# decadenza/SimpleStereo

Measured on AMD Instinct MI355X. Metric: disparity MPixels/s (H*W*nDisp per second), higher is better.
Workload: dtype f32

## Files before the change

### simplestereo_amd/csrc/asw_exact_kernels.hip.h

```cpp
#pragma once
#include "asw_shared.hip.h"
#include "lab_kernels.hip.h"
#include "glibc_math.hip.h"

namespace ssamd {

struct AswExactArgs {
    const PixRec *recL, *recR;
    const double *labL, *labR;
    const double *prox;
    u64 *keyL, *keyR;
    int16_t *disp;
    AswExactQueue q;
    AswExactQueue raw;
    double *ecost;
    u64 *costL, *costR;
    uint32_t *idxL, *idxR;
    uint32_t *wslotL, *wslotR;
    uint32_t *wpix;
    double *wtab;
    unsigned int wcap;
    int H, W, win, pad, minD, maxD, row0, rows;
    double gammaC;
};

__device__ __forceinline__ double exact_sqrt(double x)
{
#pragma clang fp contract(off)
    const double y0 = sqrt(x);
    if (!(y0 > 0.0) || !(y0 < 1.0e300)) return y0;
    const double e = fma(-y0, y0, x);
    return y0 + e / (2.0 * y0);
}

__global__ __launch_bounds__(256) void bgr2lab_f64_pair_kernel(const PixRec *__restrict__ recL, const PixRec *__restrict__ recR,
                                                               double *__restrict__ labL, double *__restrict__ labR, long long npix)
{
    SSAMD_LAB_TABLES_IN_LDS(T)
    long long q = (long long)blockIdx.x * blockDim.x + threadIdx.x;
    const long long stride = (long long)gridDim.x * blockDim.x;
    for (; q < 2 * npix; q += stride) {
        const bool right = q >= npix;
        const long long p = right ? q - npix : q;
        const uint32_t v = (right ? recR : recL)[p].bgrx;
        double L, a, b;
        bgr_to_lab_f64(v & 0xff, (v >> 8) & 0xff, (v >> 16) & 0xff, L, a, b, T);
        double *const o = (right ? labR : labL) + 3 * p;
        o[0] = L; o[1] = a; o[2] = b;
    }
}

__device__ __forceinline__ bool exact_overflowed(const AswExactArgs &A)
{
    return A.q.counter[0] > A.q.cap || (A.raw.entries && A.raw.counter[0] > A.raw.cap);
}

__global__ __launch_bounds__(256) void asw_exact_filter_kernel(const AswExactArgs A)
{
    const unsigned n = min(A.raw.counter[0], A.raw.cap);
    const unsigned nloop = (n + 255u) & ~255u;
    for (unsigned e0 = blockIdx.x * blockDim.x; e0 < nloop; e0 += gridDim.x * blockDim.x) {
        const unsigned e = e0 + threadIdx.x;
        unsigned s2 = 0;
        uint32_t pix = 0, rkey = 0xffffffffu;
        int d = 0;
        if (e < n) {
            const u64 ent = A.raw.entries[e];
            const uint32_t key = A.raw.ekeys[e];
            rkey = key;
            pix = (uint32_t)ent;
            d = (int)((ent >> 32) & 0xffff);
            const unsigned sides = (unsigned)(ent >> 48) & 3u;
            const uint32_t esc = 0xC0000000u - __float_as_uint(2.0f * A.q.sat_abs);
            if (sides & EXACT_SIDE_L) {
                const u64 g = A.keyL[pix];
                if ((int)(uint32_t)g != d && (uint32_t)(g >> 32) < esc && exact_near(key, (uint32_t)(g >> 32), A.q.tol, A.q.sat_abs, exact_zkey(A.win))) s2 |= EXACT_SIDE_L;
            }
            if ((sides & EXACT_SIDE_R) && A.keyR) {
                const u64 g = A.keyR[pix - (uint32_t)d];
                if ((uint32_t)g != pix % (uint32_t)A.W && (uint32_t)(g >> 32) < esc && exact_near(key, (uint32_t)(g >> 32), A.q.tol, A.q.sat_abs, exact_zkey(A.win))) s2 |= EXACT_SIDE_R;
            }
        }
        asw_exact_push_wave(A.q, s2 != 0, pix, d, s2, rkey);
    }
}

__global__ __launch_bounds__(256) void asw_exact_escalate_kernel(const AswExactArgs A)
{
    const AswExactQueue &Q = A.q;
    const uint32_t esc = 0xC0000000u - __float_as_uint(2.0f * Q.sat_abs);
    const long long n = (long long)A.rows * A.W;
    for (long long q = (long long)blockIdx.x * blockDim.x + threadIdx.x; q < n; q += (long long)gridDim.x * blockDim.x) {
        const int x = (int)(q % A.W);
        const u64 gl = A.keyL[q];
        if (gl != KEY_NONE && (uint32_t)(gl >> 32) >= esc) {
            const int dwin = (int)(uint32_t)gl, dhi = min(A.maxD, x);
            const int cnt = dhi - A.minD;
            if (cnt > 0) {
                unsigned slot = atomicAdd(Q.counter, (unsigned)cnt);
                for (int d = A.minD; d <= dhi; ++d)
                    if (d != dwin) {
                        if (slot < Q.cap) Q.entries[slot] = exact_entry((uint32_t)q, d, EXACT_SIDE_L);
                        ++slot;
                    }
                Q.flagL[q] = 1;
            }
        }
        if (A.keyR) {
            const u64 gr = A.keyR[q];
            if (gr != KEY_NONE && (uint32_t)(gr >> 32) >= esc) {
                const int xwin = (int)(uint32_t)gr;
                const int dhi = min(A.maxD, A.W - 1 - x), cnt = dhi - A.minD;
                if (cnt > 0) {
                    unsigned slot = atomicAdd(Q.counter, (unsigned)cnt);
                    for (int d = A.minD; d <= dhi; ++d)
                        if (x + d != xwin) {
                            if (slot < Q.cap) Q.entries[slot] = exact_entry((uint32_t)(q + d), d, EXACT_SIDE_R);
                            ++slot;
                        }
                    Q.flagR[q] = 1;
                }
            }
        }
    }
}

static constexpr int EXACT_ZSEG = 64, EXACT_ZWIN_MAX = 64;
__global__ __launch_bounds__(256) void asw_exact_zero_kernel(const AswExactArgs A)
{
    extern __shared__ __attribute__((aligned(16))) char zsmem[];
    const AswExactQueue &Q = A.q;
    const int W = A.W, H = A.H, win = A.win, p = A.pad;
    const int segs_per_row = (W + EXACT_ZSEG - 1) / EXACT_ZSEG;
    const int tid = threadIdx.x;
    const int TW = EXACT_ZSEG + 2 * p;
    uint32_t *const tA = reinterpret_cast<uint32_t *>(zsmem);
    uint32_t *const tB = tA + win * TW;
    __shared__ int s_idx[EXACT_ZSEG], s_state[EXACT_ZSEG];
    __shared__ int s_cur;
    for (long long seg = blockIdx.x; seg < (long long)A.rows * segs_per_row; seg += gridDim.x) {
        const int yr = (int)(seg / segs_per_row), x0 = (int)(seg - (long long)yr * segs_per_row) * EXACT_ZSEG, y = A.row0 + yr;
        if (!Q.zrow[yr]) continue;
        for (int side = 0; side < (A.keyR ? 2 : 1); ++side) {
            __syncthreads();
            if (tid < EXACT_ZSEG) {
                const int x = x0 + tid;
                bool z = false;
                int idx = 0;
                if (x < W) {
                    const long long q = (long long)yr * W + x;
                    if (side == 0) {
                        z = Q.zeroL[q] != 0;
                        if (z) {
                            if (A.keyL) { const u64 g = A.keyL[q]; z = g != KEY_NONE && (uint32_t)(g >> 32) == 0u; idx = (int)(uint32_t)g; }
                            else idx = (int)A.disp[q];
                        }
                    } else {
                        z = Q.zeroR[q] != 0;
                        if (z) { const u64 g = A.keyR[q]; z = g != KEY_NONE && (uint32_t)(g >> 32) == 0u; idx = (int)(uint32_t)g; }
                    }
                }
                s_idx[tid] = idx;
                s_state[tid] = z ? 1 : 0;
            }
            if (__syncthreads_or(tid < EXACT_ZSEG && s_state[tid] == 1) == 0) continue;
            if (win >= EXACT_ZWIN_MAX) {
                if (tid < EXACT_ZSEG && s_state[tid] == 1) s_state[tid] = 3;
            } else {
                const PixRec *const imgA = side ? A.recR : A.recL, *const imgB = side ? A.recL : A.recR;
                auto stage = [&](uint32_t *tile, const PixRec *img, int shift) {
                    for (int k0 = 0; k0 < win * TW; k0 += 8 * 256) {
                        uint32_t v[8];
#pragma unroll
                        for (int u = 0; u < 8; ++u) {
                            const int k = k0 + u * 256 + tid, i = k / TW, c = k - i * TW, ii = y - p + i, cc = x0 - p + c + shift;
                            v[u] = (k < win * TW && (unsigned)ii < (unsigned)H && (unsigned)cc < (unsigned)W) ? img[(size_t)ii * W + cc].bgrx : 0x80000000u;
                        }
#pragma unroll
                        for (int u = 0; u < 8; ++u) {
                            const int k = k0 + u * 256 + tid;
                            if (k < win * TW) tile[k] = v[u];
                        }
                    }
                };
                stage(tA, imgA, 0);
                for (;;) {
                    __syncthreads();
                    if (tid == 0) {
                        int cur = -1;
                        for (int k = 0; k < EXACT_ZSEG; ++k)
                            if (s_state[k] == 1) { cur = side ? s_idx[k] - (x0 + k) : s_idx[k]; break; }
                        s_cur = cur;
                    }
                    __syncthreads();
                    const int d = s_cur;
                    if (d < 0) break;
                    const int shift = side ? d : -d;
                    stage(tB, imgB, shift);
                    __syncthreads();
                    const int px = tid & (EXACT_ZSEG - 1), part = tid >> 6;
                    const bool mine = s_state[px] == 1 && (side ? s_idx[px] - (x0 + px) : s_idx[px]) == d;
                    bool nz = false;
                    if (mine) {
                        uint32_t acc = 0;
                        for (int i = part; i < win; i += 4) {
                            const uint32_t *const ra = tA + i * TW + px, *const rb = tB + i * TW + px;
#pragma unroll 8
                            for (int j = 0; j < win; ++j) {
                                const uint32_t a = ra[j], b = rb[j];
                                acc |= ((a | b) >> 31) ? 0u : (a ^ b);
                            }
                        }
                        nz = acc != 0u;
                    }
                    __syncthreads();
                    if (mine && part == 0) s_state[px] = 2;
                    __syncthreads();
                    if (mine && nz) s_state[px] = 3;
                }
            }
            __syncthreads();
            if (tid < EXACT_ZSEG && s_state[tid] == 3) {
                const int xq = x0 + tid, widx = s_idx[tid];
                const long long pq = (long long)yr * W + xq;
                if (side == 0) {
                    const int dhi = min(A.maxD, xq), cnt = dhi - A.minD;
                    if (cnt > 0) {
                        unsigned slot = atomicAdd(Q.counter, (unsigned)cnt);
                        for (int d = A.minD; d <= dhi; ++d)
                            if (d != widx) { if (slot < Q.cap) Q.entries[slot] = exact_entry((uint32_t)pq, d, EXACT_SIDE_L); ++slot; }
                        Q.flagL[pq] = 1;
                    }
                } else {
                    const int dhi = min(A.maxD, W - 1 - xq), cnt = dhi - A.minD;
                    if (cnt > 0) {
                        unsigned slot = atomicAdd(Q.counter, (unsigned)cnt);
                        for (int d = A.minD; d <= dhi; ++d)
                            if (xq + d != widx) { if (slot < Q.cap) Q.entries[slot] = exact_entry((uint32_t)(pq + d), d, EXACT_SIDE_R); ++slot; }
                        Q.flagR[pq] = 1;
                    }
                }
            }
        }
    }
}

__device__ __forceinline__ void exact_assign_wslot(const AswExactArgs &A, bool flagged, u64 mask, uint32_t pix, uint32_t side)
{
    if (mask == 0 || A.wcap == 0) return;
    const int leader = (int)__builtin_ctzll(mask);
    const unsigned lane = __builtin_amdgcn_mbcnt_hi(~0u, __builtin_amdgcn_mbcnt_lo(~0u, 0u));
    unsigned base = 0;
    if ((int)lane == leader) base = atomicAdd(A.q.counter + 6, (unsigned)__builtin_popcountll(mask));
    base = (unsigned)__builtin_amdgcn_readlane((int)base, leader);
    if (flagged) {
        const unsigned slot = base + (unsigned)__builtin_popcountll(mask & (((u64)1 << lane) - 1));
        (side ? A.wslotR : A.wslotL)[pix] = slot;
        if (slot < A.wcap) A.wpix[slot] = pix | (side << 31);
    }
}

__global__ __launch_bounds__(256) void asw_exact_winners_kernel(const AswExactArgs A)
{
    const AswExactQueue &Q = A.q;
    const long long n = (long long)A.rows * A.W;
    for (long long q0 = (long long)blockIdx.x * blockDim.x; q0 < n; q0 += (long long)gridDim.x * blockDim.x) {
        const long long q = q0 + threadIdx.x;
        const bool inb = q < n;
        const bool fl = inb && Q.flagL[q];
        if (fl) {
            A.costL[q] = ~0ull;
            A.idxL[q] = 0xffffffffu;
        }
        const int dwin = fl ? (A.keyL ? (int)(uint32_t)A.keyL[q] : (int)A.disp[q]) : 0;
        const u64 ml = __builtin_amdgcn_ballot_w64(fl);
        if (ml && fl && (int)__builtin_ctzll(ml) == (int)(threadIdx.x & 63)) atomicAdd(Q.counter + 1, (unsigned)__builtin_popcountll(ml));
        exact_assign_wslot(A, fl, ml, (uint32_t)q, 0u);
        asw_exact_push_wave(Q, fl, (uint32_t)q, dwin, EXACT_SIDE_L, fl && A.keyL ? (uint32_t)(A.keyL[q] >> 32) : 0xffffffffu);
        if (A.keyR) {
            const bool fr = inb && Q.flagR[q];
            int xl = 0, xr = 0;
            if (fr) {
                A.costR[q] = ~0ull;
                A.idxR[q] = 0xffffffffu;
                xr = (int)(q % A.W);
                xl = (int)(uint32_t)A.keyR[q];
            }
            const u64 mr = __builtin_amdgcn_ballot_w64(fr);
            if (mr && fr && (int)__builtin_ctzll(mr) == (int)(threadIdx.x & 63)) atomicAdd(Q.counter + 2, (unsigned)__builtin_popcountll(mr));
            exact_assign_wslot(A, fr, mr, (uint32_t)q, 1u);
            asw_exact_push_wave(Q, fr, (uint32_t)(q + (xl - xr)), xl - xr, EXACT_SIDE_R, fr ? (uint32_t)(A.keyR[q] >> 32) : 0xffffffffu);
        }
    }
}

__global__ __launch_bounds__(256) void asw_exact_wtab_kernel(const AswExactArgs A)
{
#pragma clang fp contract(off)
    __shared__ uint64_t s_exp[256];
    for (int k = threadIdx.x; k < 256; k += blockDim.x) s_exp[k] = gm_exp_tab[k];
    __syncthreads();
    if (exact_overflowed(A)) return;
    const unsigned n = min(A.q.counter[6], A.wcap);
    const int lane = threadIdx.x & 63, W = A.W, H = A.H, win = A.win, p = A.pad, win2 = win * win;
    for (unsigned slot = blockIdx.x * 4 + (threadIdx.x >> 6); slot < n; slot += gridDim.x * 4) {
        const uint32_t pw = A.wpix[slot], pix = pw & 0x7fffffffu;
        const double *const lab = (pw >> 31) ? A.labR : A.labL;
        const int yr = (int)(pix / (uint32_t)W), x = (int)(pix - (uint32_t)yr * (uint32_t)W), y = A.row0 + yr;
        const double *const c = lab + 3 * ((size_t)y * W + x);
        const double c0 = c[0], c1 = c[1], c2 = c[2];
        double *const out = A.wtab + (size_t)slot * win2;
        for (int t = lane; t < win2; t += 64) {
            const int i = t / win, j = t - i * win, ii = y - p + i, cc = x - p + j;
            double w = 0.0;
            if ((unsigned)ii < (unsigned)H && (unsigned)cc < (unsigned)W) {
                const double *const tp = lab + 3 * ((size_t)ii * W + cc);
                const double a0 = tp[0] - c0, a1 = tp[1] - c1, a2 = tp[2] - c2;
                w = A.prox[t] * glibc_exp_t(-exact_sqrt(a0 * a0 + a1 * a1 + a2 * a2) / A.gammaC, s_exp);
            }
            out[t] = w;
        }
    }
}

static constexpr int EXACT_WAVES = 4;
static constexpr int EXACT_CHUNK = 256;
__global__ __launch_bounds__(64 * EXACT_WAVES) void asw_exact_eval_kernel(const AswExactArgs A)
{
#pragma clang fp contract(off)
    __shared__ double s_w[EXACT_WAVES][EXACT_CHUNK], s_c[EXACT_WAVES][EXACT_CHUNK];
    __shared__ uint64_t s_exp[256];
    for (int k = threadIdx.x; k < 256; k += blockDim.x) s_exp[k] = gm_exp_tab[k];
    __syncthreads();
    if (exact_overflowed(A)) return;
    const int lane = threadIdx.x & 63, wv = threadIdx.x >> 6;
    double *const sw = s_w[wv], *const sc = s_c[wv];
    const unsigned n = min(A.q.counter[0], A.q.cap);
    const int W = A.W, H = A.H, win = A.win, p = A.pad;
    for (unsigned e = blockIdx.x * EXACT_WAVES + wv; e < n; e += gridDim.x * EXACT_WAVES) {
        const u64 ent = A.q.entries[e];
        const uint32_t pix = (uint32_t)ent;
        const int d = (int)((ent >> 32) & 0xffff);
        const unsigned sides = (unsigned)(ent >> 48) & 3u;
        const int yr = (int)(pix / (uint32_t)W), x = (int)(pix - (uint32_t)yr * (uint32_t)W);
        const int y = A.row0 + yr, xr = x - d;
        const double *const cl = A.labL + 3 * ((size_t)y * W + x), *const cr = A.labR + 3 * ((size_t)y * W + xr);
        const double cl0 = cl[0], cl1 = cl[1], cl2 = cl[2], cr0 = cr[0], cr1 = cr[1], cr2 = cr[2];
        const int jlo = max(0, p - xr), jhi = min(win, W + p - x), ncol = jhi - jlo;
        const int ilo = max(0, p - y), ihi = min(win, H + p - y);
        const int ntap = (ihi - ilo) * ncol;
        const uint32_t s1 = A.wcap && A.q.flagL && A.q.flagL[pix] ? A.wslotL[pix] : 0xffffffffu;
        const uint32_t s2 = A.wcap && A.q.flagR && A.q.flagR[pix - (uint32_t)d] ? A.wslotR[pix - (uint32_t)d] : 0xffffffffu;
        const double *const t1 = s1 < A.wcap ? A.wtab + (size_t)s1 * win * win : nullptr;
        const double *const t2 = s2 < A.wcap ? A.wtab + (size_t)s2 * win * win : nullptr;
        double acc = 0.0;
        bool all_zero = false;
        if ((unsigned)(ent >> 48) & EXACT_HINT_ZERO) {
            bool nz = false;
            for (int t = lane; t < ntap; t += 64) {
                const int q = t / ncol, i = ilo + q, j = jlo + (t - q * ncol);
                const int ii = y - p + i, jj = xr - p + j, kk = x - p + j;
                nz = nz || __builtin_amdgcn_sad_u8(A.recL[(size_t)ii * W + kk].bgrx, A.recR[(size_t)ii * W + jj].bgrx, 0u) != 0u;
            }
            all_zero = __builtin_amdgcn_ballot_w64(nz) == 0;
        }
        for (int t0 = 0; t0 < (all_zero ? 0 : ntap); t0 += EXACT_CHUNK) {
            const int nt = min(EXACT_CHUNK, ntap - t0);
            for (int t = lane; t < nt; t += 64) {
                const int q = (t0 + t) / ncol, i = ilo + q, j = jlo + (t0 + t - q * ncol);
                const int ii = y - p + i, jj = xr - p + j, kk = x - p + j;
                const double pr = A.prox[i * win + j];
                double w1, w2;
                if (t1) w1 = t1[i * win + j];
                else {
                    const double *const tl = A.labL + 3 * ((size_t)ii * W + kk);
                    const double a0 = tl[0] - cl0, a1 = tl[1] - cl1, a2 = tl[2] - cl2;
                    w1 = pr * glibc_exp_t(-exact_sqrt(a0 * a0 + a1 * a1 + a2 * a2) / A.gammaC, s_exp);
                }
                if (t2) w2 = t2[i * win + j];
                else {
                    const double *const tr = A.labR + 3 * ((size_t)ii * W + jj);
                    const double b0 = tr[0] - cr0, b1 = tr[1] - cr1, b2 = tr[2] - cr2;
                    w2 = pr * glibc_exp_t(-exact_sqrt(b0 * b0 + b1 * b1 + b2 * b2) / A.gammaC, s_exp);
                }
                const int tad = min(40, (int)__builtin_amdgcn_sad_u8(A.recL[(size_t)ii * W + kk].bgrx, A.recR[(size_t)ii * W + jj].bgrx, 0u));
                const double ww = w1 * w2;
                sw[t] = ww;
                sc[t] = ww * tad;
            }
            __builtin_amdgcn_wave_barrier();
            asm volatile("s_waitcnt lgkmcnt(0)" ::: "memory");
            if (lane < 2) {
                const double *const src = lane ? sw : sc;
                int t = 0;
                for (; t + 16 <= nt; t += 16) {
                    double v[16];
#pragma unroll
                    for (int u = 0; u < 16; ++u) v[u] = src[t + u];
#pragma unroll
                    for (int u = 0; u < 16; ++u) acc += v[u];
                }
                for (; t < nt; ++t) acc += src[t];
            }
            asm volatile("s_waitcnt lgkmcnt(0)" ::: "memory");
            __builtin_amdgcn_wave_barrier();
        }
        const double tot = __shfl(acc, 1);
        if (lane == 0) {
            const double c = all_zero ? 0.0 : acc / tot;
            A.ecost[e] = c;
            const u64 bits = (u64)__double_as_longlong(c);
            if (sides & EXACT_SIDE_L) atomicMin(A.costL + pix, bits);
            if (sides & EXACT_SIDE_R) atomicMin(A.costR + (pix - (uint32_t)d), bits);
        }
    }
}

__global__ __launch_bounds__(256) void asw_exact_resolve_kernel(const AswExactArgs A)
{
    if (exact_overflowed(A)) return;
    const unsigned n = A.q.counter[0];
    for (unsigned e = blockIdx.x * blockDim.x + threadIdx.x; e < n; e += gridDim.x * blockDim.x) {
        const u64 ent = A.q.entries[e];
        const uint32_t pix = (uint32_t)ent;
        const int d = (int)((ent >> 32) & 0xffff);
        const unsigned sides = (unsigned)(ent >> 48) & 3u;
        const u64 bits = (u64)__double_as_longlong(A.ecost[e]);
        if ((sides & EXACT_SIDE_L) && A.costL[pix] == bits) atomicMin(A.idxL + pix, (uint32_t)d);
        if ((sides & EXACT_SIDE_R) && A.costR[pix - (uint32_t)d] == bits) atomicMin(A.idxR + (pix - (uint32_t)d), pix % (uint32_t)A.W);
    }
}

__global__ __launch_bounds__(256) void asw_exact_patch_kernel(const AswExactArgs A)
{
    if (exact_overflowed(A)) return;
    const long long n = (long long)A.rows * A.W;
    for (long long q = (long long)blockIdx.x * blockDim.x + threadIdx.x; q < n; q += (long long)gridDim.x * blockDim.x) {
        if (A.q.flagL[q] && A.idxL[q] != 0xffffffffu) {
            if (A.keyL) A.keyL[q] = (A.keyL[q] & 0xffffffff00000000ull) | (u64)A.idxL[q];
            else A.disp[q] = (int16_t)A.idxL[q];
        }
        if (A.keyR && A.q.flagR[q] && A.idxR[q] != 0xffffffffu) A.keyR[q] = (A.keyR[q] & 0xffffffff00000000ull) | (u64)A.idxR[q];
    }
}

}
```

### simplestereo_amd/csrc/asw_prepass_kernels.hip.h

```cpp
#pragma once
#include "common.hip.h"
#include "lab_kernels.hip.h"

namespace ssamd {

static constexpr int TADV_COLS = 64;
template <bool BYTES>
__device__ __forceinline__ void asw_tad_tile(const void *__restrict__ srcL, const void *__restrict__ srcR, unsigned char *__restrict__ evol,
                                             int W, int pad, int minD, int Dc, int Se, int erow0, int erows, int evolW, int rd, long long npix_total,
                                             int bx, int by, int bz, char *smem)
{
    uint32_t *const sL = reinterpret_cast<uint32_t *>(smem);
    uint32_t *const sR = sL + TADV_COLS;
    const int r = erow0 + by, z = bz, uc0 = bx * TADV_COLS;
    const int P = Se >> 2, dlo = minD + z * Dc, dhi = dlo + Dc - 1;
    const int u0 = uc0 - pad, xr0 = u0 - dhi;
    auto pixel = [&](const void *src, int col) -> uint32_t {
        const size_t q = (size_t)r * W + col;
        if constexpr (BYTES) {
            typedef uint32_t __attribute__((aligned(1))) u32_unaligned;
            const uint8_t *const b = reinterpret_cast<const uint8_t *>(src) + 3 * q;
            return (long long)q + 1 < npix_total ? (*reinterpret_cast<const u32_unaligned *>(b) & 0xffffffu)
                                                 : ((uint32_t)b[0] | ((uint32_t)b[1] << 8) | ((uint32_t)b[2] << 16));
        } else {
            return reinterpret_cast<const PixRec *>(src)[q].bgrx;
        }
    };
    for (int k = threadIdx.x; k < 2 * TADV_COLS + Dc; k += blockDim.x) {
        const bool isL = k < TADV_COLS;
        const int col = isL ? u0 + k : xr0 + (k - TADV_COLS);
        const uint32_t v = (unsigned)col < (unsigned)W ? pixel(isL ? srcL : srcR, col) : 0x80000000u;
        (isL ? sL : sR)[isL ? k : k - TADV_COLS] = v;
    }
    __syncthreads();
    const int ncols = min(TADV_COLS, evolW - uc0);
    uint32_t *const out = reinterpret_cast<uint32_t *>(evol + (((size_t)z * erows + by) * (size_t)evolW + uc0) * Se);
    auto dword = [&](int c, int slot, uint32_t lp) {
        uint32_t v = 0;
        const int d0 = rd == 6 ? 6 * (slot >> 1) + 4 * (slot & 1) : 4 * slot, nv = rd == 6 && (slot & 1) ? 2 : 4;
        if (!(lp >> 31) && d0 < Dc) {
            const uint32_t *const rp = sR + c + (Dc - 1) - d0;
#pragma unroll
            for (int q = 0; q < 4; ++q) {
                const uint32_t rv = q < nv && d0 + q < Dc ? rp[-q] : 0x80000000u;
                if (!(rv >> 31)) v |= min(__builtin_amdgcn_sad_u8(lp, rv, 0u), 40u) << (8 * q);
            }
        }
        return v;
    };
    if ((P & 3) == 0) {
        const int P4 = P >> 2;
        uint4 *const out4 = reinterpret_cast<uint4 *>(out);
        for (int k = threadIdx.x; k < ncols * P4; k += blockDim.x) {
            const int c = k / P4, s4 = 4 * (k - c * P4);
            const uint32_t lp = sL[c];
            out4[k] = make_uint4(dword(c, s4, lp), dword(c, s4 + 1, lp), dword(c, s4 + 2, lp), dword(c, s4 + 3, lp));
        }
        return;
    }
    for (int k = threadIdx.x; k < ncols * P; k += blockDim.x) {
        const int c = k / P, slot = k - c * P;
        out[k] = dword(c, slot, sL[c]);
    }
}

__global__ __launch_bounds__(256) void asw_tad_volume_kernel(const PixRec *__restrict__ recL, const PixRec *__restrict__ recR,
                                                             unsigned char *__restrict__ evol, int W, int pad, int minD, int Dc,
                                                             int Se, int erow0, int erows, int evolW, int rd = 4)
{
    extern __shared__ __attribute__((aligned(16))) char smem[];
    asw_tad_tile<false>(recL, recR, evol, W, pad, minD, Dc, Se, erow0, erows, evolW, rd, 0, blockIdx.x, blockIdx.y, blockIdx.z, smem);
}

struct AswPrepassArgs {
    const uint8_t *bgrL, *bgrR;
    PixRec *recL, *recR;
    unsigned char *evol;
    long long npix_total;
    int W, pad, minD, Dc, Se, erow0, erows, evolW, rd;
    int lab_blocks, ex, ey;
};
__global__ __launch_bounds__(256) void asw_prepass_kernel(const AswPrepassArgs P)
{
    extern __shared__ __attribute__((aligned(16))) char smem[];
    if ((int)blockIdx.x < P.lab_blocks) {
        SSAMD_LAB_TABLES_IN_LDS(T)
        const long long np = (long long)P.erows * P.W, first = (long long)P.erow0 * P.W;
        const uint8_t *const bl = P.bgrL + 3 * first, *const br = P.bgrR + 3 * first;
        PixRec *const rl = P.recL + first, *const rr = P.recR + first;
        typedef uint32_t __attribute__((aligned(1))) u32_unaligned;
        for (long long q = (long long)blockIdx.x * blockDim.x + threadIdx.x; q < 2 * np; q += (long long)P.lab_blocks * blockDim.x) {
            const bool right = q >= np;
            const long long p = right ? q - np : q;
            const uint8_t *const bgr = right ? br : bl;
            uint32_t B, G, R;
            if (p + 1 < np) {
                const uint32_t v = *reinterpret_cast<const u32_unaligned *>(bgr + 3 * p);
                B = v & 0xff; G = (v >> 8) & 0xff; R = (v >> 16) & 0xff;
            } else {
                B = bgr[3 * p]; G = bgr[3 * p + 1]; R = bgr[3 * p + 2];
            }
            PixRec o;
            bgr_to_lab(B, G, R, o.L, o.a, o.b, T);
            o.bgrx = B | (G << 8) | (R << 16);
            (right ? rr : rl)[p] = o;
        }
        return;
    }
    const int b = (int)blockIdx.x - P.lab_blocks, bx = b % P.ex, by = (b / P.ex) % P.ey, bz = b / (P.ex * P.ey);
    asw_tad_tile<true>(P.bgrL, P.bgrR, P.evol, P.W, P.pad, P.minD, P.Dc, P.Se, P.erow0, P.erows, P.evolW, P.rd, P.npix_total, bx, by, bz, smem);
}

}
```

### simplestereo_amd/csrc/host_asw.h

```cpp
namespace {
template <class T> int get_prox_table(TableCache &tc, const char *what, int win, double gammaP, hipStream_t s, const T **out)
{
    return get_table(tc, win, gammaP, (size_t)win * win, what, s, out, [&](T *host) {
        const int p = win / 2;
        for (int i = 0; i < win; ++i)
            for (int j = 0; j < win; ++j) {
                const double di = i - p, dj = j - p;
                host[(size_t)i * win + j] = (T)glibc_exp(-std::sqrt(di * di + dj * dj) / gammaP);
            }
    });
}
int get_prox(Ctx &c, int win, double gammaP, hipStream_t s, const float **out) { return get_prox_table(c.proxTabs, "proximity table", win, gammaP, s, out); }
int get_prox64(Ctx &c, int win, double gammaP, hipStream_t s, const double **out) { return get_prox_table(c.proxTabs64, "fp64 proximity table", win, gammaP, s, out); }

int reset_keys(DevBuf &keys, size_t nout, hipStream_t s)
{
    if (int rc = keys.reserve(nout * 8)) return rc;
    HIP_TRY(hipMemsetAsync(keys.ptr, 0xFF, nout * 8, s));
    return SSAMD_OK;
}

int launch_finalize(Ctx &c, int slot, bool lrcheck, int b0, int nb, int W, int16_t *d_disp, hipStream_t s,
                    int16_t *d_raw_right = nullptr)
{
    if (nb <= 0) return SSAMD_OK;
    const size_t off = (size_t)b0 * W;
    const long long n = (long long)nb * W;
    const int blocks = (int)std::min<long long>((n + 255) / 256, 256 * 8);
    Timed t(c, s, slot);
    if (d_raw_right) {
        hipLaunchKernelGGL(wta_decode_kernel, dim3(blocks), dim3(256), 0, s, (const u64 *)c.keyL.ptr + off, d_disp + off, nb, W, 0);
        hipLaunchKernelGGL(wta_decode_kernel, dim3(blocks), dim3(256), 0, s, (const u64 *)c.keyR.ptr + off, d_raw_right + off, nb, W, 1);
    } else if (lrcheck) {
        const size_t lds = (((size_t)W * 2 + 15) & ~(size_t)15) + W;
        int rc = grant_dyn_lds(c, (const void *)lr_check_fill_kernel, (int)lds);
        if (rc) return rc;
        hipLaunchKernelGGL(lr_check_fill_kernel, dim3(nb), dim3(256), lds, s, (const u64 *)c.keyL.ptr + off,
                           (const u64 *)c.keyR.ptr + off, d_disp + off, nb, W);
    } else {
        hipLaunchKernelGGL(wta_decode_kernel, dim3(blocks), dim3(256), 0, s, (const u64 *)c.keyL.ptr + off, d_disp + off, nb, W, 0);
    }
    HIP_TRY(hipGetLastError());
    return SSAMD_OK;
}

using AswKernel = void (*)(const AswArgs);
using AswWaveKernel = void (*)(const AswWaveArgs);
struct AswPipeVariant { bool costs; int SL, SR, Se; AswKernel kernel; };
const AswPipeVariant kPipeVariants[] = {
#define SSAMD_PIPE_INSTANCE(C, SL, SR, SE) {C, SL, SR, SE, asw_aggregate_pipe_kernel<C, SL, SR, SE>},
#include "asw_instances.inc"
#undef SSAMD_PIPE_INSTANCE
};
struct AswWaveVariant { int RD; bool costs; int RX, KL, KR, KM; bool creg; AswWaveKernel kernel; };
#define SSAMD_WAVE_VARIANT(RX, KL, KR, KM, CREG) {4, false, RX, KL, KR, KM, CREG, asw_aggregate_wave_kernel<false, RX, KL, KR, KM, CREG>}
const AswWaveVariant kWaveVariants[] = {
#define SSAMD_WAVE6_INSTANCE(C, K, CREG) {6, C, 4, 0, 0, K, CREG, asw_aggregate_wave6_kernel<C, K, CREG>},
#include "asw_instances.inc"
#undef SSAMD_WAVE6_INSTANCE
    SSAMD_WAVE_VARIANT(4, 0, 0, 2, false), SSAMD_WAVE_VARIANT(4, 0, 0, 2, true),
    SSAMD_WAVE_VARIANT(4, 0, 0, 3, false), SSAMD_WAVE_VARIANT(4, 0, 0, 3, true),
    SSAMD_WAVE_VARIANT(4, 0, 0, 4, false), SSAMD_WAVE_VARIANT(4, 0, 0, 4, true),
    SSAMD_WAVE_VARIANT(8, 0, 0, 2, false), SSAMD_WAVE_VARIANT(8, 0, 0, 3, false), SSAMD_WAVE_VARIANT(8, 0, 0, 4, false),
    SSAMD_WAVE_VARIANT(8, 2, 2, 0, false),
    SSAMD_WAVE_VARIANT(8, 1, 2, 0, false),
    SSAMD_WAVE_VARIANT(4, 1, 2, 0, false),
    SSAMD_WAVE_VARIANT(4, 2, 2, 0, false),
    SSAMD_WAVE_VARIANT(4, 2, 3, 0, false),
};
#undef SSAMD_WAVE_VARIANT

AswKernel asw_pick_pipe_kernel(const AswGeom &g, bool costs, int asw_static)
{
    AswKernel pk = nullptr;
    for (const AswPipeVariant &v : kPipeVariants) {
        if (v.costs != costs) continue;
        if (v.SL == 0 && !pk) pk = v.kernel;
        if (asw_static != 0 && v.SL == g.SL && v.SR == g.SR && v.Se == g.Se) pk = v.kernel;
    }
    return pk;
}

AswWaveKernel asw_pick_wave_kernel(const AswWaveGeom &g, bool costs, bool unrolled)
{
    const bool straight = unrolled && !costs;
    const int kl = g.merged ? 0 : (g.Txw + 63) / 64, kr = g.merged ? 0 : (g.nRcw + 63) / 64, km = g.merged ? g.K : 0;
    for (const AswWaveVariant &v : kWaveVariants)
        if (straight && v.RD == g.RD && !v.costs && v.RX == g.RX && v.KL == kl && v.KR == kr && v.KM == km && v.creg == (g.creg != 0)) return v.kernel;
    if (g.RD == 6) return costs ? asw_aggregate_wave6_kernel<true, 0> : asw_aggregate_wave6_kernel<false, 0>;
    return g.RX == 8 ? (costs ? asw_aggregate_wave_kernel<true, 8> : asw_aggregate_wave_kernel<false, 8>)
                     : (costs ? asw_aggregate_wave_kernel<true, 4> : asw_aggregate_wave_kernel<false, 4>);
}

struct MatchCall {
    const uint8_t *dL = nullptr, *dR = nullptr;
    const RemapSrc *rm = nullptr;
    int H = 0, W = 0, row0 = 0, rows = 0;
    int win = 0, maxD = 0, minD = 0;
    int16_t *d_disp = nullptr;
    hipStream_t s = nullptr;
};
struct AswCall : MatchCall {
    int skip_at = 0, skip = 0;
    double gammaC = 0, gammaP = 0;
    bool consistent = false, alternate = false, exact = false;
    float *d_costs = nullptr;
    int16_t *d_raw_right = nullptr;
};

AswCall asw_call(const uint8_t *dL, const uint8_t *dR, int H, int W, int row0, int rows, int win, int maxD, int minD, double gammaC,
                 double gammaP, int consistent, int16_t *d_disp, void *stream, bool alternate = false, bool exact = false)
{
    AswCall q;
    q.dL = dL; q.dR = dR; q.H = H; q.W = W; q.row0 = row0; q.rows = rows;
    q.win = win; q.maxD = maxD; q.minD = minD; q.gammaC = gammaC; q.gammaP = gammaP; q.consistent = consistent != 0;
    q.d_disp = d_disp; q.s = (hipStream_t)stream; q.alternate = alternate; q.exact = exact;
    return q;
}

struct AswRun : AswCall {
    Ctx &c;
    const Tuning &t;
    PlanOptions po;
    int p, nD, grows, r0, r1, lab_blocks;
    size_t nout;
    long long np2;
    ShapeKey shape;
    AswGeom geom;
    std::vector<AswGeom> trial;
    bool need_keys = false, lab_pending = false;
    size_t evol_cap_max = 0, evol_limit = 0;
    const float *d_prox = nullptr;
    const unsigned char *evol = nullptr;
    int evolW = 0;
    AswWaveGeom wave;
    AswExactQueue xq_final{}, xq_raw{}, xq_kernel{};
};

bool asw_is_direct(const AswRun &r, const AswGeom &g) { return r.nD >= 1 && (g.nchunks == 1 || g.wave_rx) && !r.consistent; }

int asw_check_call(const AswCall &q)
{
    int rc = check_common(q.H, q.W, q.win, q.minD, q.maxD, q.row0, q.rows);
    if (rc) return rc;
    if (q.skip < 0 || q.skip_at < 0 || q.skip_at + q.skip > q.rows) return fail(SSAMD_EINVAL, "bad row gap [%d,%d) in a range of %d rows", q.skip_at, q.skip_at + q.skip, q.rows);
    if (q.skip > 0 && (q.alternate || q.d_costs || q.d_raw_right)) return fail(SSAMD_EINVAL, "two row ranges: plain, consistent and exact matching only");
    if (q.skip == q.rows) return 1;
    if (!(q.gammaC > 0) || !(q.gammaP > 0)) return fail(SSAMD_EINVAL, "gammaC and gammaP must be positive");
    if (q.exact && (q.alternate || q.d_costs)) return fail(SSAMD_EINVAL, "the exact (fp64 tie-break) mode has no alternate-rows form and no cost dump");
    if (q.alternate && q.d_costs) return fail(SSAMD_EINVAL, "the alternate-rows mode has no cost dump");
    return q.rows == 0 ? 1 : SSAMD_OK;
}

bool asw_volume_fits(AswRun &r, size_t bytes)
{
    if (bytes > r.evol_cap_max) return false;
    if (bytes <= r.c.evol.cap) return true;
    if (!r.evol_limit) {
        size_t free_b = 0, total_b = 0;
        r.evol_limit = r.evol_cap_max;
        if (hipMemGetInfo(&free_b, &total_b) == hipSuccess) r.evol_limit = std::min(r.evol_cap_max, r.c.evol.cap + free_b / 2);
        else (void)hipGetLastError();
    }
    return bytes <= r.evol_limit;
}

bool asw_wave_volume_fits(AswRun &r, const AswGeom &g)
{
    AswWaveGeom wg;
    if (!g.wave_rx || !asw_wave_layout(wg, r.po, r.win, r.nD, g.wave_rx)) return !g.wave_rx;
    const int xt = (r.W + wg.Txw - 1) / wg.Txw, erows = std::min(r.H, r.row0 + r.rows + r.win / 2) - std::max(0, r.row0 - r.win / 2);
    return asw_volume_fits(r, (size_t)erows * (size_t)round_up(xt * wg.Txw + 2 * (r.win / 2), 4) * (size_t)wg.Se + 4096);
}

int asw_plan_call(AswRun &r)
{
    if (r.nD >= 1)
        if (int rc = asw_choose_geometry(r.geom, r.po, r.W, r.grows, r.win, r.nD)) return rc;
    const double call_taps = (double)r.W * r.grows * r.nD * r.win * r.win;
    if (autotune_due(g_asw_geom, r.shape, call_taps) && r.nD >= 1 && !asw_geometry_forced(r.t)) {
        AswGeom tmp;
        if (asw_search(tmp, r.po, r.W, r.grows, r.win, r.nD, &r.trial) != SSAMD_OK || r.trial.size() < 2) r.trial.clear();
    }
    r.evol_cap_max = r.t.evol_max_mb ? std::min((size_t)24 << 30, (size_t)r.t.evol_max_mb << 20) : (size_t)24 << 30;
    if (r.nD >= 1 && r.geom.wave_rx && !asw_wave_volume_fits(r, r.geom)) ++r.c.evol_fallbacks;
    if (r.nD >= 1 && !asw_wave_volume_fits(r, r.geom)) r.geom.wave_rx = 0;
    r.trial.erase(std::remove_if(r.trial.begin(), r.trial.end(), [&](const AswGeom &g) { return !asw_wave_volume_fits(r, g); }), r.trial.end());
    if (r.trial.size() < 2) r.trial.clear();
    r.need_keys = !asw_is_direct(r, r.geom) || r.alternate;
    for (const AswGeom &g : r.trial) r.need_keys = r.need_keys || !asw_is_direct(r, g);
    return SSAMD_OK;
}

int asw_lab_records(AswRun &r)
{
    Ctx &c = r.c;
    Timed t(c, r.s, SSAMD_K_LAB);
    if (r.rm)
        hipLaunchKernelGGL(remap_lab_records_pair_kernel, dim3(r.lab_blocks), dim3(256), 0, r.s, *r.rm, (PixRec *)c.recL.ptr, (PixRec *)c.recR.ptr,
                           (long long)r.r0 * r.W, r.np2);
    else
        hipLaunchKernelGGL(bgr2lab_records_pair_kernel, dim3(r.lab_blocks), dim3(256), 0, r.s, r.dL + (size_t)r.r0 * r.W * 3, r.dR + (size_t)r.r0 * r.W * 3,
                           (PixRec *)c.recL.ptr + (size_t)r.r0 * r.W, (PixRec *)c.recR.ptr + (size_t)r.r0 * r.W, r.np2);
    HIP_TRY(hipGetLastError());
    return SSAMD_OK;
}

int asw_prepare_volume(AswRun &r, const AswGeom &g)
{
    Ctx &c = r.c;
    hipStream_t s = r.s;
    r.evol = nullptr;
    int chunks = g.nchunks, Tx = g.Tx, Dc = g.Dc, Se = g.Se;
    if (g.wave_rx) {
        if (!asw_wave_layout(r.wave, r.po, r.win, r.nD, g.wave_rx, !r.d_costs && r.t.wave_unroll != 0))
            return fail(SSAMD_ELIMIT, "wave kernel geometry does not fit LDS");
        chunks = 1; Tx = r.wave.Txw; Dc = r.wave.Dc; Se = r.wave.Se;
    } else if (!g.pipe || r.t.asw_evol == 0) {
        return SSAMD_OK;
    }
    const int xt = (r.W + Tx - 1) / Tx, erows = r.r1 - r.r0;
    const int evolW = round_up(xt * Tx + 2 * r.p + (g.wave_rx ? 0 : Tx / 2 + 8), 4);
    const size_t bytes = (size_t)chunks * (size_t)erows * (size_t)evolW * (size_t)Se;
    if (c.evol.cap > ((size_t)256 << 20) && (bytes + 4096) * 4 < c.evol.cap) {
        if (r.trial.empty() && ++c.evol_small_calls >= 8) {
            (void)hipStreamSynchronize(s);
            c.evol.release();
            c.evol_small_calls = 0;
        }
    } else {
        c.evol_small_calls = 0;
    }
    int erc = SSAMD_ENOMEM;
    if (r.t.evol_fail) {
        void *none = nullptr;
        size_t free_b = 0, total_b = (size_t)512 << 30;
        (void)hipMemGetInfo(&free_b, &total_b);
        if (hipMalloc(&none, 2 * total_b) == hipSuccess) (void)hipFree(none);
    } else if (asw_volume_fits(r, bytes + 4096)) {
        erc = c.evol.reserve(bytes + 4096);
    }
    if (erc) {
        (void)hipGetLastError();
        if (g.wave_rx) return fail(erc == SSAMD_ENOMEM ? SSAMD_ENOMEM : erc, "TAD volume of %zu bytes does not fit the device memory left", bytes);
        ++c.evol_fallbacks;
        g_err.clear();
        return SSAMD_OK;
    }
    r.evol = (const unsigned char *)c.evol.ptr;
    r.evolW = evolW;
    const int rd = g.wave_rx ? r.wave.RD : 4;
    Timed t(c, s, SSAMD_K_LAB);
    const dim3 egrid((unsigned)((evolW + TADV_COLS - 1) / TADV_COLS), (unsigned)erows, (unsigned)chunks);
    const size_t elds = (size_t)(2 * TADV_COLS + Dc) * 4;
    const long long tiles = (long long)egrid.x * egrid.y * egrid.z;
    if (r.lab_pending && tiles + r.lab_blocks < (1ll << 31)) {
        AswPrepassArgs pa;
        pa.bgrL = r.dL; pa.bgrR = r.dR; pa.recL = (PixRec *)c.recL.ptr; pa.recR = (PixRec *)c.recR.ptr;
        pa.evol = (unsigned char *)c.evol.ptr; pa.npix_total = (long long)r.H * r.W;
        pa.W = r.W; pa.pad = r.p; pa.minD = r.minD; pa.Dc = Dc; pa.Se = Se; pa.erow0 = r.r0; pa.erows = erows; pa.evolW = evolW;
        pa.rd = rd;
        pa.lab_blocks = r.lab_blocks; pa.ex = (int)egrid.x; pa.ey = (int)egrid.y;
        if (int grc = grant_dyn_lds(c, (const void *)asw_prepass_kernel, (int)elds)) return grc;
        hipLaunchKernelGGL(asw_prepass_kernel, dim3((unsigned)(tiles + r.lab_blocks)), dim3(256), elds, s, pa);
        HIP_TRY(hipGetLastError());
        r.lab_pending = false;
        return SSAMD_OK;
    }
    if (r.lab_pending) {
        r.lab_pending = false;
        if (int lrc = asw_lab_records(r)) return lrc;
    }
    if (int grc = grant_dyn_lds(c, (const void *)asw_tad_volume_kernel, (int)elds)) return grc;
    hipLaunchKernelGGL(asw_tad_volume_kernel, egrid, dim3(256), elds, s, (const PixRec *)c.recL.ptr, (const PixRec *)c.recR.ptr,
                       (unsigned char *)c.evol.ptr, r.W, r.p, r.minD, Dc, Se, r.r0, erows, evolW, rd);
    HIP_TRY(hipGetLastError());
    return SSAMD_OK;
}

template <class Args> void asw_fill_args(Args &x, const AswRun &r, const AswGeom &g)
{
    const bool direct = asw_is_direct(r, g);
    x.recL = (const PixRec *)r.c.recL.ptr; x.recR = (const PixRec *)r.c.recR.ptr;
    x.prox = r.d_prox;
    x.keyL = direct ? nullptr : (u64 *)r.c.keyL.ptr;
    x.keyR = r.consistent ? (u64 *)r.c.keyR.ptr : nullptr;
    x.disp = direct ? r.d_disp : nullptr;
    x.costs = r.d_costs;
    x.cost_keys = 0;
    x.xq = r.xq_kernel;
    x.evol = r.evol; x.erow0 = r.r0; x.erows = r.r1 - r.r0; x.evolW = r.evolW;
    x.H = r.H; x.W = r.W; x.win = r.win; x.pad = r.p; x.minD = r.minD; x.maxD = r.maxD; x.row0 = r.row0; x.rows = r.rows;
    x.kC = (float)(-1.4426950408889634 / r.gammaC);
    x.ystep = r.alternate ? 2 : 1;
    x.yb0 = 0;
    x.yskip_at = r.skip > 0 ? r.skip_at : 0x7fffffff; x.yskip = r.skip;
}

int asw_launch_pipe(AswRun &r, const AswArgs &a, const dim3 &grid)
{
    Ctx &c = r.c;
    const AswGeom &g = a.g;
    const AswKernel pk = asw_pick_pipe_kernel(g, r.d_costs != nullptr, r.t.asw_static);
    const int pipe_lds = a.evol ? g.lds_bytes_evol : g.lds_bytes;
    if (pipe_lds > 160 * 1024) return fail(SSAMD_ELIMIT, "this tile needs the TAD volume (LDS %d bytes without it)", pipe_lds);
    if (int grc = grant_dyn_lds(c, (const void *)pk, pipe_lds)) return grc;
    int rows_main = r.grows;
    AswGeom tail_g;
    const int per_simd = (g.threads / 64 + 3) / 4;
    const long long resident = std::max(1, std::min(3 / std::max(1, per_simd), (160 * 1024) / std::max(1, pipe_lds)));
    const long long per_row = (long long)grid.x * g.nchunks, slots = (long long)c.cus * resident;
    if (!r.alternate && r.t.asw_tail != 0 && g.XG >= 4) {
        const long long n = per_row * r.grows;
        const long long full = n / slots, rem = n - full * slots;
        if (full >= 1 && rem > 0 && 2 * rem <= slots && (full < 32 || r.t.asw_tail > 0)) {
            const int rm = (int)(full * slots / per_row);
            if (rm >= 1 && rm < r.grows &&
                asw_layout_e(tail_g, r.po, r.win, (g.XG + 1) / 2, g.DG, 160 * 1024, g.JC, 8, true, false, true) && tail_g.pipe &&
                tail_g.Se == g.Se && tail_g.Dc == g.Dc &&
                (a.evol == nullptr || round_up(((r.W + tail_g.Tx - 1) / tail_g.Tx) * tail_g.Tx + 2 * r.p, 4) <= a.evolW)) {
                tail_g.nchunks = g.nchunks;
                rows_main = rm;
            }
        }
    }
    const long long items = per_row * rows_main;
    long long workers = r.t.asw_persist > 0 ? std::min<long long>(r.t.asw_persist, slots) : (r.t.asw_persist < 0 && items >= 64 * slots ? slots : 0);
    workers = std::min(workers, items);
    if (workers > 0 && items < (1ll << 30)) {
        const size_t pq_bytes = (size_t)(ASW_PQ_QUEUES + 1) * ASW_PQ_LINE * 4;
        if (!c.pq.ptr) {
            if (int prc = c.pq.reserve(pq_bytes)) return prc;
            HIP_TRY(hipMemsetAsync(c.pq.ptr, 0, pq_bytes, r.s));
        }
        HIP_TRY(hipMemsetAsync(c.pq.ptr, 0, (size_t)ASW_PQ_QUEUES * ASW_PQ_LINE * 4, r.s));
        AswArgs pa = a;
        pa.pq = (unsigned int *)c.pq.ptr;
        pa.pq_nx = (int)grid.x; pa.pq_ny = rows_main; pa.pq_items = (int)items;
        ++c.persist_launches;
        hipLaunchKernelGGL(pk, dim3((unsigned)workers), dim3(g.threads), pipe_lds, r.s, pa);
    } else {
        hipLaunchKernelGGL(pk, dim3(grid.x, rows_main, grid.z), dim3(g.threads), pipe_lds, r.s, a);
    }
    HIP_TRY(hipGetLastError());
    if (rows_main < r.grows) {
        ++c.tail_splits;
        AswArgs t = a;
        t.g = tail_g;
        t.yb0 = rows_main;
        const AswKernel tk = asw_pick_pipe_kernel(tail_g, r.d_costs != nullptr, 0);
        const int tail_lds = a.evol ? tail_g.lds_bytes_evol : tail_g.lds_bytes;
        if (int grc = grant_dyn_lds(c, (const void *)tk, tail_lds)) return grc;
        hipLaunchKernelGGL(tk, dim3((r.W + tail_g.Tx - 1) / tail_g.Tx, r.grows - rows_main, tail_g.nchunks), dim3(tail_g.threads),
                           tail_lds, r.s, t);
        HIP_TRY(hipGetLastError());
    }
    return SSAMD_OK;
}

int asw_launch(AswRun &r, const AswGeom &g)
{
    r.geom = g;
    if (g.wave_rx) {
        AswWaveArgs wa;
        asw_fill_args(wa, r, g);
        wa.g = r.wave;
        const AswWaveKernel wk = asw_pick_wave_kernel(wa.g, r.d_costs != nullptr, r.t.wave_unroll != 0);
        const int lds = wa.g.wave_lds * wa.g.waves, xt = (r.W + wa.g.Txw - 1) / wa.g.Txw;
        if (int grc = grant_dyn_lds(r.c, (const void *)wk, lds)) return grc;
        hipLaunchKernelGGL(wk, dim3((xt + wa.g.waves - 1) / wa.g.waves, r.grows, 1), dim3(64 * wa.g.waves), lds, r.s, wa);
        HIP_TRY(hipGetLastError());
        return SSAMD_OK;
    }
    AswArgs a{};
    asw_fill_args(a, r, g);
    a.g = g;
    const dim3 grid((r.W + g.Tx - 1) / g.Tx, r.grows, g.nchunks);
    if (g.pipe) return asw_launch_pipe(r, a, grid);
    const bool chunked = g.JC < r.win;
    AswKernel kern = chunked ? (r.d_costs ? asw_aggregate_kernel<true, true> : asw_aggregate_kernel<false, true>)
                             : (r.d_costs ? asw_aggregate_kernel<true, false> : asw_aggregate_kernel<false, false>);
    if (g.Rx == 4)
        kern = chunked ? (r.d_costs ? asw_aggregate_kernel<true, true, 4> : asw_aggregate_kernel<false, true, 4>)
                       : (r.d_costs ? asw_aggregate_kernel<true, false, 4> : asw_aggregate_kernel<false, false, 4>);
    if (int grc = grant_dyn_lds(r.c, (const void *)kern, g.lds_bytes)) return grc;
    hipLaunchKernelGGL(kern, grid, dim3(g.threads), g.lds_bytes, r.s, a);
    HIP_TRY(hipGetLastError());
    return SSAMD_OK;
}

int asw_autotune(AswRun &r)
{
    hipStream_t s = r.s;
    hipEvent_t e0 = nullptr, e1 = nullptr;
    HIP_TRY(hipEventCreate(&e0));
    HIP_TRY(hipEventCreate(&e1));
    bool all_prepared = true;
    const bool want_evol = r.t.asw_evol != 0;
    for (const AswGeom &g : r.trial) {
        if (asw_prepare_volume(r, g) != SSAMD_OK) { all_prepared = false; continue; }
        if (g.pipe && !g.wave_rx && want_evol && !r.evol) all_prepared = false;
        if (asw_launch(r, g) != SSAMD_OK) all_prepared = false;
    }
    const int fastest = autotune_rounds(r.trial.size(), 4, false, e0, e1, s, &all_prepared, [&](size_t ci) {
        const AswGeom &g = r.trial[ci];
        const bool launched = asw_prepare_volume(r, g) == SSAMD_OK && asw_launch(r, g) == SSAMD_OK;
        if (g.pipe && !g.wave_rx && want_evol && !r.evol) all_prepared = false;
        return launched;
    });
    if (fastest >= 0) r.geom = r.trial[fastest];
    (void)hipEventDestroy(e0);
    (void)hipEventDestroy(e1);
    if (all_prepared) autotune_keep(g_asw_geom, r.shape, r.geom);
    else g_err.clear();
    return SSAMD_OK;
}

int asw_final_volume(AswRun &r, AswGeom &final_geom)
{
    int rc = asw_prepare_volume(r, final_geom);
    if (rc == SSAMD_ENOMEM && final_geom.wave_rx) {
        ++r.c.evol_fallbacks;
        g_err.clear();
        final_geom.wave_rx = 0;
        r.geom = final_geom;
        if (!asw_is_direct(r, final_geom) && !r.need_keys) {
            if ((rc = reset_keys(r.c.keyL, r.nout, r.s))) return rc;
            r.need_keys = true;
        }
        rc = asw_prepare_volume(r, final_geom);
    }
    if (rc) return rc;
    if (final_geom.pipe && !final_geom.wave_rx && !r.evol && final_geom.lds_bytes > 160 * 1024) {
        AswGeom g2;
        if ((rc = asw_search(g2, PlanOptions{r.t, true}, r.W, r.grows, r.win, r.nD))) return rc;
        g2.wave_rx = 0;
        if (!asw_is_direct(r, g2) && !r.need_keys && (rc = reset_keys(r.c.keyL, r.nout, r.s))) return rc;
        final_geom = g2;
        if ((rc = asw_prepare_volume(r, final_geom))) return rc;
    }
    return SSAMD_OK;
}

int asw_alternate_fill(AswRun &r)
{
    Ctx &c = r.c;
    hipStream_t s = r.s;
    int rc;
    AswAltArgs f;
    const size_t nodd = (size_t)(r.rows / 2) * r.W;
    if ((double)nodd * ((r.nD + 7) / 8 + 1) >= 4.0e9)
        return fail(SSAMD_ELIMIT, "alternate-rows mode: image x disparity range too large for the 32-bit job counter");
    f.cap = (unsigned int)std::min<size_t>(std::max<size_t>(nodd, 1 << 16), 1u << 28);
    if (r.t.alt_queue_cap)
        f.cap = (unsigned int)r.t.alt_queue_cap;
    if ((rc = c.altq.reserve((size_t)f.cap * 8 + 16))) return rc;
    f.ctr = (unsigned int *)c.altq.ptr; f.queue = (u64 *)((char *)c.altq.ptr + 16);
    HIP_TRY(hipMemsetAsync(f.ctr, 0, 16, s));
    f.recL = (const PixRec *)c.recL.ptr; f.recR = (const PixRec *)c.recR.ptr; f.prox = r.d_prox;
    f.disp = r.d_disp; f.key = (u64 *)c.keyL.ptr;
    f.H = r.H; f.W = r.W; f.win = r.win; f.pad = r.p; f.minD = r.minD; f.maxD = r.maxD; f.row0 = r.row0; f.rows = r.rows;
    f.kC = (float)(-1.4426950408889634 / r.gammaC);
    const dim3 pix_grid((r.W + 255) / 256, r.rows / 2);
    Timed t(c, s, SSAMD_K_ASW_ALT);
    hipLaunchKernelGGL(asw_alt_scan_kernel, pix_grid, dim3(256), 0, s, f);
    hipLaunchKernelGGL(asw_alt_jobs_kernel, dim3(256 * 8), dim3(256), 0, s, f);
    hipLaunchKernelGGL(asw_alt_decode_kernel, pix_grid, dim3(256), 0, s, f);
    HIP_TRY(hipGetLastError());
    return SSAMD_OK;
}

int asw_device_impl(Ctx &c, const AswCall &q)
{
    int rc = asw_check_call(q);
    if (rc) return rc > 0 ? SSAMD_OK : rc;
    hipStream_t s = q.s;
    ScratchOrder order(c, s);
    const Tuning &t = tune();
    AswRun r{q, c, t, PlanOptions{t, false}};
    r.exact = q.exact && q.maxD >= q.minD;
    r.p = q.win / 2; r.nD = q.maxD - q.minD + 1;
    r.nout = (size_t)q.rows * q.W;
    r.grows = q.alternate ? (q.rows + 1) / 2 : q.rows - q.skip;
    r.shape = {q.W, r.grows, q.win, r.nD};
    r.r0 = std::max(0, q.row0 - r.p); r.r1 = std::min(q.H, q.row0 + q.rows + r.p);
    r.np2 = (long long)(r.r1 - r.r0) * q.W;
    r.lab_blocks = (int)std::min<long long>((2 * r.np2 + 255) / 256, 256 * 8);
    if ((rc = asw_plan_call(r))) return rc;
    if (r.need_keys && (rc = reset_keys(c.keyL, r.nout, s))) return rc;
    if (q.consistent && (rc = reset_keys(c.keyR, r.nout, s))) return rc;
    if (r.nD >= 1) {
        if ((rc = c.recL.reserve((size_t)q.H * q.W * sizeof(PixRec)))) return rc;
        if ((rc = c.recR.reserve((size_t)q.H * q.W * sizeof(PixRec)))) return rc;
        if ((rc = get_prox(c, q.win, q.gammaP, s, &r.d_prox))) return rc;
        r.lab_pending = r.trial.empty() && !q.rm && t.prepass_fuse != 0;
        if (!r.lab_pending && (rc = asw_lab_records(r))) return rc;
        if (!r.trial.empty() && (rc = asw_autotune(r))) return rc;
        AswGeom final_geom = r.geom;
        if ((rc = asw_final_volume(r, final_geom))) return rc;
        if (r.lab_pending) {
            r.lab_pending = false;
            if ((rc = asw_lab_records(r))) return rc;
        }
        if (r.exact) {
            if (!r.trial.empty()) {
                if (r.need_keys && (rc = reset_keys(c.keyL, r.nout, s))) return rc;
                if (q.consistent && (rc = reset_keys(c.keyR, r.nout, s))) return rc;
            }
            if ((rc = asw_exact_prepare(c, q.W, q.rows, q.win, r.nD, q.gammaC, q.consistent, asw_is_direct(r, final_geom), s, r.xq_final, r.xq_raw, r.xq_kernel))) return rc;
        }
        Timed agg(c, s, SSAMD_K_ASW_AGG);
        if ((rc = asw_launch(r, final_geom))) return rc;
    }
    const bool direct = asw_is_direct(r, r.geom);
    if (r.exact && r.nD >= 1 &&
        (rc = asw_exact_pass(c, r.xq_final, r.xq_raw, q.H, q.W, q.row0, q.rows, q.win, q.maxD, q.minD, q.gammaC, q.gammaP, q.consistent, direct, q.d_disp, s)))
        return rc;
    if (!direct && q.skip > 0) {
        if ((rc = launch_finalize(c, SSAMD_K_ASW_FIN, q.consistent, 0, q.skip_at, q.W, q.d_disp, s)) ||
            (rc = launch_finalize(c, SSAMD_K_ASW_FIN, q.consistent, q.skip_at + q.skip, q.rows - q.skip_at - q.skip, q.W, q.d_disp, s)))
            return rc;
    } else if (!direct && (rc = launch_finalize(c, SSAMD_K_ASW_FIN, q.consistent, 0, q.rows, q.W, q.d_disp, s, q.d_raw_right))) return rc;
    return q.alternate && q.rows > 1 ? asw_alternate_fill(r) : SSAMD_OK;
}

int asw_alternate_rows(Ctx &c, AswCall q, int row_parity)
{
    int rc = check_common(q.H, q.W, q.win, q.minD, q.maxD, q.row0, q.rows);
    if (rc) return rc;
    if (q.rows == 0) return SSAMD_OK;
    const int row0 = q.row0, rows = q.rows;
    const bool top_odd = ((row0 + row_parity) & 1) != 0, bottom_odd = ((row0 + rows - 1 + row_parity) & 1) != 0;
    if (top_odd && row0 == 0)
        return fail(SSAMD_EINVAL, "alternate rows: the first output row is an odd row of the image, the sub-image must start at least one row above it");
    const int e0 = top_odd ? row0 - 1 : row0, e1 = bottom_odd ? std::min(q.H, row0 + rows + 1) : row0 + rows;
    q.alternate = true;
    if (e0 == row0 && e1 == row0 + rows) return asw_device_impl(c, q);
    ScratchOrder order(c, q.s);
    if ((rc = c.altdisp.reserve((size_t)(e1 - e0) * q.W * 2))) return rc;
    int16_t *const d_disp = q.d_disp;
    q.row0 = e0; q.rows = e1 - e0; q.d_disp = (int16_t *)c.altdisp.ptr;
    if ((rc = asw_device_impl(c, q))) return rc;
    HIP_TRY(hipMemcpyAsync(d_disp, (const int16_t *)c.altdisp.ptr + (size_t)(row0 - e0) * q.W, (size_t)rows * q.W * 2, hipMemcpyDeviceToDevice, q.s));
    return SSAMD_OK;
}
}
```

### simplestereo_amd/csrc/host_asw_exact.h

```cpp
namespace {
int get_prox64(Ctx &c, int win, double gammaP, hipStream_t s, const double **out);

int asw_exact_prepare(Ctx &c, int W, int rows, int win, int nD, double gammaC, bool consistent, bool direct, hipStream_t s,
                      AswExactQueue &q, AswExactQueue &raw, AswExactQueue &kernel_q)
{
    const size_t nout = (size_t)rows * W;
    if (nout >= ((size_t)1 << 32)) return fail(SSAMD_ELIMIT, "exact mode: more than 2^32 output pixels per call");
    const size_t all_cands = 2 * (nout * (size_t)nD + nout);
    size_t cap = std::min<size_t>(std::max<size_t>(4 * nout, std::min<size_t>(all_cands, (size_t)1 << 23)), (size_t)1 << 26);
    if (tune().exact_cap) cap = (size_t)tune().exact_cap;
    size_t rawcap = direct ? 0 : std::min<size_t>(std::max<size_t>(2 * nout, std::min<size_t>(all_cands, (size_t)1 << 23)), (size_t)1 << 26);
    if (!direct && tune().exact_cap) rawcap = std::max<size_t>(rawcap, cap);
    if (!direct && tune().exact_rawcap) rawcap = (size_t)tune().exact_rawcap;
    int rc;
    if ((rc = c.xqueue.reserve(cap * 8)) || (rc = c.xcost.reserve(cap * 8)) || (rc = c.xflags.reserve(64 + 4 * nout + (size_t)rows)) ||
        (rc = c.xslots.reserve(nout * 32)) || (rawcap && (rc = c.xraw.reserve(rawcap * 12))))
        return rc;
    c.xcap = (unsigned int)cap;
    c.xrawcap = (unsigned int)rawcap;
    HIP_TRY(hipMemsetAsync(c.xflags.ptr, 0, 64 + 4 * nout + (size_t)rows, s));
    q.entries = (u64 *)c.xqueue.ptr;
    q.ekeys = nullptr;
    q.counter = (unsigned int *)c.xflags.ptr;
    q.flagL = (unsigned char *)c.xflags.ptr + 64;
    q.flagR = consistent ? q.flagL + nout : nullptr;
    q.zeroL = q.flagL + 2 * nout;
    q.zeroR = consistent ? q.flagL + 3 * nout : nullptr;
    q.zrow = q.flagL + 4 * nout;
    q.W = (unsigned int)W;
    q.cap = (unsigned int)cap;
    q.tol = (uint32_t)std::min(1.0e6, (double)tune().exact_tol * std::max(1.0, 5.0 / gammaC) * std::max(1.0, win / 35.0));
    q.sat_abs = (float)(1.5 * 2.0 * 2.0 * ((double)win * win + 3.0) * 1.1102230246251565e-16 * 40.0);
    q.deep = 0xffffffffu;
    raw = AswExactQueue{};
    if (!direct) {
        raw = q;
        union { float f; uint32_t u; } sa; sa.f = q.sat_abs;
        raw.deep = 0xC0000000u - sa.u;
        raw.entries = (u64 *)c.xraw.ptr;
        raw.ekeys = (uint32_t *)((u64 *)c.xraw.ptr + rawcap);
        raw.counter = q.counter + 4;
        raw.flagL = raw.flagR = nullptr;
        raw.cap = (unsigned int)rawcap;
    }
    kernel_q = direct ? q : raw;
    return SSAMD_OK;
}

int asw_exact_pass(Ctx &c, const AswExactQueue &q, const AswExactQueue &raw, int H, int W, int row0, int rows, int win, int maxD, int minD, double gammaC, double gammaP,
                   bool consistent, bool direct, int16_t *d_disp, hipStream_t s)
{
    const int p = win / 2;
    const size_t nout = (size_t)rows * W, npix = (size_t)H * W;
    int rc;
    const double *d_prox = nullptr;
    if ((rc = get_prox64(c, win, gammaP, s, &d_prox))) return rc;
    if ((rc = c.xlabL.reserve(npix * 24)) || (rc = c.xlabR.reserve(npix * 24))) return rc;
    AswExactArgs x;
    x.recL = (const PixRec *)c.recL.ptr; x.recR = (const PixRec *)c.recR.ptr;
    x.labL = (const double *)c.xlabL.ptr; x.labR = (const double *)c.xlabR.ptr;
    x.prox = d_prox;
    x.keyL = direct ? nullptr : (u64 *)c.keyL.ptr; x.keyR = consistent ? (u64 *)c.keyR.ptr : nullptr;
    x.disp = d_disp;
    x.q = q;
    x.raw = raw;
    x.ecost = (double *)c.xcost.ptr;
    x.costL = (u64 *)c.xslots.ptr; x.costR = x.costL + nout;
    x.idxL = (uint32_t *)(x.costR + nout); x.idxR = x.idxL + nout;
    x.wslotL = x.idxR + nout; x.wslotR = x.wslotL + nout;
    {
        const size_t per = (size_t)win * win * 8;
        size_t wcap = std::min<size_t>(65536, ((size_t)64 << 20) / per);
        if (nout >= ((size_t)1 << 31)) wcap = 0;
        if (wcap && (rc = c.xwtab.reserve(wcap * 8 + wcap * per))) return rc;
        x.wcap = (unsigned int)wcap;
        x.wpix = (uint32_t *)c.xwtab.ptr;
        x.wtab = (double *)((char *)c.xwtab.ptr + wcap * 8);
    }
    x.H = H; x.W = W; x.win = win; x.pad = p; x.minD = minD; x.maxD = maxD; x.row0 = row0; x.rows = rows;
    x.gammaC = gammaC;
    Timed t(c, s, SSAMD_K_ASW_EXACT);
    {
        const int r0 = std::max(0, row0 - p), r1 = std::min(H, row0 + rows + p);
        const long long np2 = (long long)(r1 - r0) * W;
        const int blocks = (int)std::min<long long>((2 * np2 + 255) / 256, 256 * 8);
        hipLaunchKernelGGL(bgr2lab_f64_pair_kernel, dim3(blocks), dim3(256), 0, s, x.recL + (size_t)r0 * W, x.recR + (size_t)r0 * W,
                           (double *)c.xlabL.ptr + 3 * (size_t)r0 * W, (double *)c.xlabR.ptr + 3 * (size_t)r0 * W, np2);
    }
    const int pb = (int)std::min<long long>(((long long)nout + 255) / 256, 256 * 8);
    if (raw.entries) {
        hipLaunchKernelGGL(asw_exact_filter_kernel, dim3(256 * 8), dim3(256), 0, s, x);
        hipLaunchKernelGGL(asw_exact_escalate_kernel, dim3(pb), dim3(256), 0, s, x);
    }
    {
        const int zwin = std::min(win, EXACT_ZWIN_MAX - 1);
        const size_t zlds = (size_t)2 * zwin * (EXACT_ZSEG + 2 * (zwin / 2)) * 4;
        if ((rc = grant_dyn_lds(c, (const void *)asw_exact_zero_kernel, (int)zlds))) return rc;
        const long long segs = (long long)rows * ((W + EXACT_ZSEG - 1) / EXACT_ZSEG);
        hipLaunchKernelGGL(asw_exact_zero_kernel, dim3((unsigned)std::min<long long>(segs, 256 * 64)), dim3(256), zlds, s, x);
    }
    hipLaunchKernelGGL(asw_exact_winners_kernel, dim3(pb), dim3(256), 0, s, x);
    if (x.wcap) hipLaunchKernelGGL(asw_exact_wtab_kernel, dim3(256 * 4), dim3(256), 0, s, x);
    hipLaunchKernelGGL(asw_exact_eval_kernel, dim3((unsigned)(c.cus * 5)), dim3(64 * EXACT_WAVES), 0, s, x);
    hipLaunchKernelGGL(asw_exact_resolve_kernel, dim3(256 * 4), dim3(256), 0, s, x);
    hipLaunchKernelGGL(asw_exact_patch_kernel, dim3(pb), dim3(256), 0, s, x);
    HIP_TRY(hipGetLastError());
    ++c.exact_calls;
    return SSAMD_OK;
}

int asw_exact_counters(Ctx &c, unsigned int (&ctr)[5])
{
    std::fill(ctr, ctr + 5, 0u);
    if (!c.xflags.ptr || c.exact_calls == 0) return SSAMD_OK;
    HIP_TRY(hipDeviceSynchronize());
    HIP_TRY(hipMemcpy(ctr, c.xflags.ptr, sizeof(ctr), hipMemcpyDeviceToHost));
    return SSAMD_OK;
}
}
```

### simplestereo_amd/csrc/host_context.h

```cpp
namespace {
thread_local std::string g_err;

int fail(int code, const char *fmt, ...)
{
    char buf[512];
    va_list ap;
    va_start(ap, fmt);
    vsnprintf(buf, sizeof(buf), fmt, ap);
    va_end(ap);
    g_err = buf;
    return code;
}

#include "ssamd_options.h"
#include "asw_plan.h"
#include "gsw_plan.h"
#include "ftp_plan.h"
#include "np_unwrap_plan.h"

std::mutex g_tune_mutex;
std::atomic<unsigned> g_tune_version{1};

std::map<std::string, std::string> g_tuning_env;
Tuning tuning_from_env()
{
    Tuning t;
    for (const char *n : kTuningNames)
        if (const char *v = getenv(n)) {
            g_tuning_env[n] = v;
            (void)tuning_assign(t, n, v);
        }
    return t;
}
Tuning g_tuning = tuning_from_env();

const Tuning &tune()
{
    thread_local Tuning snap;
    thread_local unsigned seen = 0;
    const unsigned v = g_tune_version.load(std::memory_order_acquire);
    if (v != seen) {
        std::lock_guard<std::mutex> lk(g_tune_mutex);
        snap = g_tuning;
        seen = v;
    }
    return snap;
}

#define HIP_TRY(expr)                                                                              \
    do {                                                                                           \
        hipError_t e_ = (expr);                                                                    \
        if (e_ != hipSuccess)                                                                      \
            return fail(e_ == hipErrorOutOfMemory ? SSAMD_ENOMEM : SSAMD_EHIP, "%s failed: %s",    \
                        #expr, hipGetErrorString(e_));                                             \
    } while (0)

struct DevBuf {
    void *ptr = nullptr;
    size_t cap = 0;
    int reserve(size_t bytes)
    {
        if (bytes <= cap) return SSAMD_OK;
        if (ptr) { (void)hipFree(ptr); ptr = nullptr; cap = 0; }
        size_t want = bytes + bytes / 8 + 256;
        hipError_t e = hipMalloc(&ptr, want);
        if (e != hipSuccess) {
            ptr = nullptr;
            (void)hipGetLastError();
            return fail(SSAMD_ENOMEM, "hipMalloc(%zu) failed: %s", want, hipGetErrorString(e));
        }
        cap = want;
        return SSAMD_OK;
    }
    void release()
    {
        if (ptr) (void)hipFree(ptr);
        ptr = nullptr; cap = 0;
    }
};

struct Profile {
    bool on = false;
    struct Pair { hipEvent_t a, b; int slot; };
    std::vector<Pair> pending;
    std::vector<hipEvent_t> pool;
    double ms[SSAMD_K_COUNT] = {0};
    long long n[SSAMD_K_COUNT] = {0};
    hipEvent_t get()
    {
        if (!pool.empty()) { hipEvent_t e = pool.back(); pool.pop_back(); return e; }
        hipEvent_t e = nullptr;
        (void)hipEventCreate(&e);
        return e;
    }
    void drain()
    {
        for (auto &p : pending) {
            float t = 0.f;
            if (hipEventSynchronize(p.b) == hipSuccess && hipEventElapsedTime(&t, p.a, p.b) == hipSuccess) {
                ms[p.slot] += t;
                n[p.slot] += 1;
            }
            pool.push_back(p.a);
            pool.push_back(p.b);
        }
        pending.clear();
    }
};

struct TableEntry {
    int k0 = 0; double k1 = 0;
    DevBuf dev;
    std::vector<unsigned char> host;
};
struct TableCache {
    std::list<TableEntry> entries;
    size_t max_entries;
    explicit TableCache(size_t n) : max_entries(n) {}
    TableEntry *find(int k0, double k1)
    {
        for (auto it = entries.begin(); it != entries.end(); ++it)
            if (it->k0 == k0 && it->k1 == k1) {
                entries.splice(entries.begin(), entries, it);
                return &entries.front();
            }
        return nullptr;
    }
};

struct Ctx {
    std::mutex mu;
    int dev = -1;
    int cus = 256;
    bool lut_ready = false;
    hipStream_t stream = nullptr;
    DevBuf imgL, imgR, recL, recR, keyL, keyR, disp, costs, lab, altq, evol, altdisp;
    DevBuf xlabL, xlabR, xflags, xqueue, xcost, xslots, xctr, xraw, xwtab;
    DevBuf pq;
    DevBuf uwIn, uwOut;
    DevBuf ftpBand, ftpPhase;
    std::map<int, DevBuf> ftpTabs;
    DevBuf ftpRefTab;
    bool ftpRefTabReady = false;
    int32_t *ftpBandHost = nullptr;
    size_t ftpBandHostCap = 0;
    hipEvent_t ftp_band_copied = nullptr;
    unsigned int xcap = 0, xrawcap = 0;
    TableCache proxTabs{8}, gswTabs{4}, proxTabs64{8};
    std::map<const void *, int> max_dyn_lds;
    hipEvent_t scratch_free = nullptr;
    int evol_small_calls = 0;
    long long evol_fallbacks = 0;
    long long tail_splits = 0;
    long long exact_calls = 0;
    long long persist_launches = 0;
    long long gsw_plain_calls = 0;
    Profile prof;
};

Ctx g_ctx[16];

struct DeviceGuard {
    int saved = -1;
    DeviceGuard() { if (hipGetDevice(&saved) != hipSuccess) saved = -1; }
    ~DeviceGuard() { if (saved >= 0) (void)hipSetDevice(saved); }
    DeviceGuard(const DeviceGuard &) = delete;
    DeviceGuard &operator=(const DeviceGuard &) = delete;
};

struct Timed {
    Ctx &c; hipStream_t s; int slot; hipEvent_t a = nullptr, b = nullptr;
    Timed(Ctx &c_, hipStream_t s_, int slot_) : c(c_), s(s_), slot(slot_)
    {
        if (c.prof.on) { a = c.prof.get(); b = c.prof.get(); (void)hipEventRecord(a, s); }
    }
    ~Timed()
    {
        if (a) { (void)hipEventRecord(b, s); c.prof.pending.push_back({a, b, slot}); }
    }
};

struct CtxLock {
    DeviceGuard guard;
    std::unique_lock<std::mutex> lk;
    Ctx *c = nullptr;
    Ctx *operator->() { return c; }
    Ctx &operator*() { return *c; }
};

int get_ctx(int device, CtxLock &out)
{
    int n = 0;
    if (hipGetDeviceCount(&n) != hipSuccess || n <= 0)
        return fail(SSAMD_ENODEVICE, "no HIP device visible: libssamd has no CPU fallback");
    if (device < 0) device = out.guard.saved >= 0 ? out.guard.saved : 0;
    if (device >= n || device >= 16) return fail(SSAMD_EINVAL, "device ordinal %d out of range (%d visible)", device, n);
    HIP_TRY(hipSetDevice(device));
    Ctx &c = g_ctx[device];
    out.lk = std::unique_lock<std::mutex>(c.mu);
    out.c = &c;
    if (c.dev < 0) {
        c.dev = device;
        int cus = 0;
        if (hipDeviceGetAttribute(&cus, hipDeviceAttributeMultiprocessorCount, device) == hipSuccess && cus > 0) c.cus = cus;
        else (void)hipGetLastError();
        HIP_TRY(hipStreamCreateWithFlags(&c.stream, hipStreamNonBlocking));
        HIP_TRY(hipEventCreateWithFlags(&c.scratch_free, hipEventDisableTiming));
    }
    if (!c.lut_ready) {
        float lut[256];
        for (int v = 0; v < 256; ++v) {
            float x = v / 255.0;
            if (x > 0.04045) x = glibc_powf_pos((float)((x + 0.055) / 1.055), (float)2.4);
            else x /= 12.92;
            x *= 100;
            lut[v] = x;
        }
        HIP_TRY(hipMemcpyToSymbol(HIP_SYMBOL(c_lin100), lut, sizeof(lut)));
        c.lut_ready = true;
    }
    return SSAMD_OK;
}

int grant_dyn_lds(Ctx &c, const void *kernel, int bytes)
{
    int &granted = c.max_dyn_lds[kernel];
    if (bytes <= granted || bytes <= 48 * 1024) return SSAMD_OK;
    HIP_TRY(hipFuncSetAttribute(kernel, hipFuncAttributeMaxDynamicSharedMemorySize, bytes));
    granted = bytes;
    return SSAMD_OK;
}

struct ScratchOrder {
    Ctx &c; hipStream_t s;
    ScratchOrder(Ctx &c_, hipStream_t s_) : c(c_), s(s_) { (void)hipStreamWaitEvent(s, c.scratch_free, 0); }
    ~ScratchOrder() { (void)hipEventRecord(c.scratch_free, s); }
};

int check_common(int H, int W, int win, int minD, int maxD, int row0, int rows)
{
    if (H <= 0 || W <= 0) return fail(SSAMD_EINVAL, "Wrong image dimensions!");
    if (!(win > 0 && win % 2 == 1)) return fail(SSAMD_EINVAL, "winSize must be a positive odd number!");
    if (minD < 0) return fail(SSAMD_EINVAL, "minDisparity must be >= 0 (negative values are undefined behaviour in the reference)");
    if (W > 32767 || maxD > 32767) return fail(SSAMD_ELIMIT, "width / maxDisparity exceed the int16 disparity range");
    if (row0 < 0 || rows < 0 || row0 + rows > H) return fail(SSAMD_EINVAL, "output row range [%d,%d) outside the image (height %d)", row0, row0 + rows, H);
    if (win > 255) return fail(SSAMD_ELIMIT, "winSize %d > 255 not supported", win);
    if (rows > 65535) return fail(SSAMD_ELIMIT, "more than 65535 output rows per call: split the image into row strips");
    return SSAMD_OK;
}

template <class T, class Fill>
int get_table(TableCache &tc, int k0, double k1, size_t n, const char *what, hipStream_t s, const T **out, Fill fill)
{
    if (TableEntry *e = tc.find(k0, k1)) { *out = (const T *)e->dev.ptr; return SSAMD_OK; }
    if (tc.entries.size() >= tc.max_entries) {
        HIP_TRY(hipDeviceSynchronize());
        (void)hipFree(tc.entries.back().dev.ptr);
        tc.entries.pop_back();
    }
    tc.entries.emplace_front();
    TableEntry &e = tc.entries.front();
    e.k0 = k0; e.k1 = k1;
    e.host.resize(n * sizeof(T));
    fill(reinterpret_cast<T *>(e.host.data()));
    int rc = e.dev.reserve(n * sizeof(T));
    if (rc) { tc.entries.pop_front(); return rc; }
    hipError_t he = hipMemcpyAsync(e.dev.ptr, e.host.data(), n * sizeof(T), hipMemcpyHostToDevice, s);
    if (he != hipSuccess) {
        (void)hipFree(e.dev.ptr);
        tc.entries.pop_front();
        return fail(SSAMD_EHIP, "hipMemcpyAsync(%s) failed: %s", what, hipGetErrorString(he));
    }
    *out = (const T *)e.dev.ptr;
    return SSAMD_OK;
}

struct HostIn { DevBuf Ctx::*buf; const void *host; size_t bytes; size_t at = 0; };
struct HostOut { DevBuf Ctx::*buf; void *host; size_t bytes; size_t at = 0; };
inline char *staged(Ctx &c, DevBuf Ctx::*buf, size_t at = 0) { return (char *)(c.*buf).ptr + at; }

template <class Launch>
int host_route(int device, std::initializer_list<HostIn> in, const HostOut &out, Launch launch)
{
    CtxLock c;
    int rc = get_ctx(device, c);
    if (rc) return rc;
    for (const HostIn &i : in)
        if ((rc = ((*c).*i.buf).reserve(i.at + i.bytes))) return rc;
    if ((rc = ((*c).*out.buf).reserve(out.at + out.bytes))) return rc;
    hipStream_t s = c->stream;
    ScratchOrder order(*c, s);
    for (const HostIn &i : in) HIP_TRY(hipMemcpyAsync(staged(*c, i.buf, i.at), i.host, i.bytes, hipMemcpyHostToDevice, s));
    if ((rc = launch(*c, s))) return rc;
    HIP_TRY(hipMemcpyAsync(out.host, staged(*c, out.buf, out.at), out.bytes, hipMemcpyDeviceToHost, s));
    HIP_TRY(hipStreamSynchronize(s));
    return SSAMD_OK;
}
}
```

### simplestereo_amd/csrc/host_debug.h

```cpp
namespace {
extern "C" __global__ void debug_libm_kernel(int which, int n, const void *in, void *out)
{
    const int i = blockIdx.x * blockDim.x + threadIdx.x;
    if (i >= n) return;
    if (which == 0) reinterpret_cast<double *>(out)[i] = glibc_exp(reinterpret_cast<const double *>(in)[i]);
    else if (which == 1) reinterpret_cast<float *>(out)[i] = glibc_powf_pos(reinterpret_cast<const float *>(in)[i], (float)(1 / 3.0));
    else if (which == 2) reinterpret_cast<double *>(out)[i] = ssamd::exact_sqrt(reinterpret_cast<const double *>(in)[i]);
    else reinterpret_cast<double *>(out)[i] = reinterpret_cast<const double *>(in)[i] / 0.7 + reinterpret_cast<const double *>(in)[i] / 5.0;
}
}

extern "C" {
int ssamd_bgr2lab(const uint8_t *img, int height, int width, float *lab, int device)
{
    if (!img || !lab || height <= 0 || width <= 0) return fail(SSAMD_EINVAL, "bad argument");
    const size_t npix = (size_t)height * width;
    return host_route(device, {{&Ctx::imgL, img, npix * 3}}, {&Ctx::lab, lab, npix * 12}, [&](Ctx &c, hipStream_t s) {
        const int blocks = (int)std::min<size_t>((npix + 255) / 256, 256 * 8);
        hipLaunchKernelGGL(bgr2lab_f32_kernel, dim3(blocks), dim3(256), 0, s, (const uint8_t *)c.imgL.ptr, (float *)c.lab.ptr, (long long)npix);
        HIP_TRY(hipGetLastError());
        return SSAMD_OK;
    });
}

int ssamd_debug_exact_costs(const uint8_t *img1, const uint8_t *img2, int height, int width, int winSize, double gammaC, double gammaP,
                            int n, const int *yxd, double *costs, double *lab1, double *lab2)
{
    if (!img1 || !img2 || !yxd || !costs || n < 0) return fail(SSAMD_EINVAL, "NULL buffer");
    int rc = check_common(height, width, winSize, 0, 0, 0, height);
    if (rc) return rc;
    CtxLock c;
    if ((rc = get_ctx(-1, c))) return rc;
    const size_t npix = (size_t)height * width;
    hipStream_t s = c->stream;
    ScratchOrder order(*c, s);
    if ((rc = c->imgL.reserve(npix * 3)) || (rc = c->imgR.reserve(npix * 3)) || (rc = c->recL.reserve(npix * sizeof(PixRec))) ||
        (rc = c->recR.reserve(npix * sizeof(PixRec))) || (rc = c->xlabL.reserve(npix * 24)) || (rc = c->xlabR.reserve(npix * 24)) ||
        (rc = c->xqueue.reserve((size_t)std::max(n, 1) * 8)) || (rc = c->xcost.reserve((size_t)std::max(n, 1) * 8)) || (rc = c->xctr.reserve(64)))
        return rc;
    HIP_TRY(hipMemcpyAsync(c->imgL.ptr, img1, npix * 3, hipMemcpyHostToDevice, s));
    HIP_TRY(hipMemcpyAsync(c->imgR.ptr, img2, npix * 3, hipMemcpyHostToDevice, s));
    const int blocks = (int)std::min<long long>((2 * (long long)npix + 255) / 256, 256 * 8);
    hipLaunchKernelGGL(bgr2lab_records_pair_kernel, dim3(blocks), dim3(256), 0, s, (const uint8_t *)c->imgL.ptr, (const uint8_t *)c->imgR.ptr,
                       (PixRec *)c->recL.ptr, (PixRec *)c->recR.ptr, (long long)npix);
    hipLaunchKernelGGL(bgr2lab_f64_pair_kernel, dim3(blocks), dim3(256), 0, s, (const PixRec *)c->recL.ptr, (const PixRec *)c->recR.ptr,
                       (double *)c->xlabL.ptr, (double *)c->xlabR.ptr, (long long)npix);
    std::vector<u64> ent((size_t)n);
    for (int k = 0; k < n; ++k) {
        const int y = yxd[3 * k], x = yxd[3 * k + 1], d = yxd[3 * k + 2];
        if (y < 0 || y >= height || x < 0 || x >= width || d < 0 || x - d < 0) return fail(SSAMD_EINVAL, "candidate %d outside the image", k);
        ent[k] = (u64)((uint32_t)y * (uint32_t)width + (uint32_t)x) | ((u64)(uint32_t)d << 32);
    }
    const unsigned int ctr[16] = {(unsigned int)n};
    HIP_TRY(hipMemcpyAsync(c->xqueue.ptr, ent.data(), (size_t)n * 8, hipMemcpyHostToDevice, s));
    HIP_TRY(hipMemcpyAsync(c->xctr.ptr, ctr, sizeof(ctr), hipMemcpyHostToDevice, s));
    const double *d_prox = nullptr;
    if ((rc = get_prox64(*c, winSize, gammaP, s, &d_prox))) return rc;
    AswExactArgs x{};
    x.recL = (const PixRec *)c->recL.ptr; x.recR = (const PixRec *)c->recR.ptr;
    x.labL = (const double *)c->xlabL.ptr; x.labR = (const double *)c->xlabR.ptr;
    x.prox = d_prox; x.q.entries = (u64 *)c->xqueue.ptr; x.q.counter = (unsigned int *)c->xctr.ptr; x.q.cap = (unsigned int)std::max(n, 1);
    x.ecost = (double *)c->xcost.ptr;
    x.H = height; x.W = width; x.win = winSize; x.pad = winSize / 2; x.row0 = 0; x.rows = height; x.gammaC = gammaC;
    hipLaunchKernelGGL(asw_exact_eval_kernel, dim3(256), dim3(64 * EXACT_WAVES), 0, s, x);
    HIP_TRY(hipGetLastError());
    HIP_TRY(hipMemcpyAsync(costs, c->xcost.ptr, (size_t)n * 8, hipMemcpyDeviceToHost, s));
    if (lab1) HIP_TRY(hipMemcpyAsync(lab1, c->xlabL.ptr, npix * 24, hipMemcpyDeviceToHost, s));
    if (lab2) HIP_TRY(hipMemcpyAsync(lab2, c->xlabR.ptr, npix * 24, hipMemcpyDeviceToHost, s));
    HIP_TRY(hipStreamSynchronize(s));
    return SSAMD_OK;
}

int ssamd_debug_exact_queue(int which, long long max_n, unsigned long long *entries, unsigned int *keys, long long *n)
{
    if (!n || max_n < 0 || (max_n > 0 && !entries)) return fail(SSAMD_EINVAL, "bad argument");
    CtxLock c;
    int rc = get_ctx(-1, c);
    if (rc) return rc;
    *n = 0;
    unsigned int ctr[5];
    if ((rc = asw_exact_counters(*c, ctr))) return rc;
    const unsigned int cnt = which ? ctr[4] : ctr[0], cap = which ? c->xrawcap : c->xcap;
    *n = cnt;
    const size_t m = (size_t)std::min<long long>(std::min<unsigned int>(cnt, cap), max_n);
    if (m == 0) return SSAMD_OK;
    const void *src = which ? c->xraw.ptr : c->xqueue.ptr;
    if (!src) return SSAMD_OK;
    HIP_TRY(hipMemcpy(entries, src, m * 8, hipMemcpyDeviceToHost));
    if (which && keys) HIP_TRY(hipMemcpy(keys, (const char *)src + (size_t)c->xrawcap * 8, m * 4, hipMemcpyDeviceToHost));
    return SSAMD_OK;
}

int ssamd_debug_libm(int which, int n, const void *in, void *out)
{
    if (!in || !out || n < 0 || which < 0 || which > 3)
        return fail(SSAMD_EINVAL, "ssamd_debug_libm: which = 0 (exp, doubles), 1 (powf(x, 1/3), floats), 2 (sqrt, doubles), 3 (x / 0.7 + x / 5.0, doubles)");
    if (n == 0) return SSAMD_OK;
    const size_t bytes = (size_t)n * (which == 1 ? 4 : 8);
    return host_route(-1, {{&Ctx::lab, in, bytes, bytes}}, {&Ctx::lab, out, bytes}, [&](Ctx &c, hipStream_t s) {
        hipLaunchKernelGGL(debug_libm_kernel, dim3((n + 255) / 256), dim3(256), 0, s, which, n, (const void *)staged(c, &Ctx::lab, bytes),
                           (void *)staged(c, &Ctx::lab));
        HIP_TRY(hipGetLastError());
        return SSAMD_OK;
    });
}

int ssamd_debug_gsw_sqrt(int n, float *out)
{
    int what = 0;
    if (n < 0) { what = 1; n = -n; }
    if (!out || n <= 0 || n > GSW_TAB_SIZE) return fail(SSAMD_EINVAL, "bad argument");
    return host_route(-1, {}, {&Ctx::lab, out, (size_t)n * 4}, [&](Ctx &c, hipStream_t s) {
        hipLaunchKernelGGL(gsw_sqrt_probe_kernel, dim3((n + 255) / 256), dim3(256), 0, s, (float *)c.lab.ptr, n, what);
        HIP_TRY(hipGetLastError());
        return SSAMD_OK;
    });
}
}
```

### simplestereo_amd/csrc/host_library.h

```cpp
namespace {
int check_geometry_query(int width, int winSize, int maxDisparity, int minDisparity, const int *out, int *nD)
{
    if (!out) return fail(SSAMD_EINVAL, "out is NULL");
    int rc = check_common(1 << 14, width, winSize, minDisparity, maxDisparity, 0, 0);
    if (rc) return rc;
    *nD = maxDisparity - minDisparity + 1;
    return *nD < 1 ? fail(SSAMD_EINVAL, "empty disparity range") : SSAMD_OK;
}
}

extern "C" {
int ssamd_abi_version(void) { return SSAMD_ABI_VERSION; }
const char *ssamd_last_error(void) { return g_err.c_str(); }

int ssamd_device_count(void)
{
    int n = 0;
    if (hipGetDeviceCount(&n) != hipSuccess) return 0;
    return n;
}

const char *ssamd_kernel_name(int slot)
{
    static const char *names[SSAMD_K_COUNT] = {"asw pre-pass (asw_prepass_kernel: Lab records + TAD volume; or bgr2lab_records_pair_kernel, asw_tad_volume_kernel)", "asw aggregation kernel (asw_aggregate_pipe / _wave / asw_aggregate_kernel)",
                                               "asw finalize (wta_decode / lr_check_fill)",
                                               "gsw_aggregate_kernel", "gsw finalize (lr_check_fill)", "remap_bgr_kernel / ftp_reference_kernel", "reproject_kernel / ftp_cloud_kernel",
                                               "asw_alt_fill_kernel", "asw fp64 tie-break pass (bgr2lab_f64_pair + asw_exact_winners / _eval / _resolve / _patch kernels)",
                                               "iir_unwrap_kernel", "ftp_phase_kernel", "np_unwrap_row_kernel / np_unwrap_col_kernel"};
    return (slot >= 0 && slot < SSAMD_K_COUNT) ? names[slot] : "";
}

int ssamd_set_option(const char *name, const char *value)
{
    if (!name) return fail(SSAMD_EINVAL, "option name is NULL");
    std::lock_guard<std::mutex> lk(g_tune_mutex);
    if (value) {
        if (!tuning_assign(g_tuning, name, value)) return fail(SSAMD_EINVAL, "unknown option %s", name);
    } else {
        const auto it = g_tuning_env.find(name);
        if (!tuning_assign(g_tuning, name, it == g_tuning_env.end() ? nullptr : it->second.c_str()))
            return fail(SSAMD_EINVAL, "unknown option %s", name);
    }
    if (std::string(name) == "SSAMD_AUTOTUNE")
        g_autotune.store(g_tuning.autotune_env != -2 ? g_tuning.autotune_env : -1);
    g_tune_version.fetch_add(1, std::memory_order_release);
    return SSAMD_OK;
}

int ssamd_counter(int device, const char *name, long long *value)
{
    if (!name || !value) return fail(SSAMD_EINVAL, "name / value is NULL");
    CtxLock c;
    int rc = get_ctx(device, c);
    if (rc) return rc;
    const std::string n(name);
    if (n == "evol_fallbacks") *value = c->evol_fallbacks;
    else if (n == "evol_bytes") *value = (long long)c->evol.cap;
    else if (n == "tail_splits") *value = c->tail_splits;
    else if (n == "exact_calls") *value = c->exact_calls;
    else if (n == "pipe_persist_launches") *value = c->persist_launches;
    else if (n == "gsw_plain_calls") *value = c->gsw_plain_calls;
    else if (n == "pipe_persist_items") {
        unsigned long long done = 0;
        if (c->pq.ptr) {
            HIP_TRY(hipDeviceSynchronize());
            HIP_TRY(hipMemcpy(&done, (const unsigned int *)c->pq.ptr + ASW_PQ_QUEUES * ASW_PQ_LINE, sizeof(done), hipMemcpyDeviceToHost));
        }
        *value = (long long)done;
    }
    else if (n == "exact_entries" || n == "exact_flagged_left" || n == "exact_flagged_right" || n == "exact_overflow" || n == "exact_raw_entries") {
        unsigned int ctr[5];
        if ((rc = asw_exact_counters(*c, ctr))) return rc;
        *value = n == "exact_entries" ? ctr[0] : n == "exact_flagged_left" ? ctr[1] : n == "exact_flagged_right" ? ctr[2] :
                 n == "exact_raw_entries" ? ctr[4] : ((ctr[0] > c->xcap || (c->xrawcap && ctr[4] > c->xrawcap)) ? 1 : 0);
    }
    else return fail(SSAMD_EINVAL, "unknown counter %s", name);
    return SSAMD_OK;
}

int ssamd_autotune(int on)
{
    return g_autotune.exchange(on > 0 ? 1 : (on < 0 ? -1 : 0));
}

int ssamd_asw_geometry(int width, int rows, int winSize, int maxDisparity, int minDisparity, int *out)
{
    int nD, rc = check_geometry_query(width, winSize, maxDisparity, minDisparity, out, &nD);
    if (rc) return rc;
    const Tuning &t = tune();
    const PlanOptions po{t, false};
    AswGeom g;
    if ((rc = asw_choose_geometry(g, po, width, rows, winSize, nD))) return rc;
    out[0] = g.Tx; out[1] = g.Dc; out[2] = g.nchunks; out[3] = g.threads; out[4] = g.lds_bytes;
    out[5] = (width + g.Tx - 1) / g.Tx; out[6] = rows; out[7] = g.nchunks;
    AswWaveGeom wg;
    if (g.wave_rx && asw_wave_layout(wg, po, winSize, nD, g.wave_rx, t.wave_unroll != 0)) {
        out[0] = wg.Txw * wg.waves; out[1] = wg.Dc; out[2] = 1; out[3] = 64 * wg.waves; out[4] = wg.wave_lds * wg.waves;
        out[5] = (width + out[0] - 1) / out[0]; out[7] = 1;
    }
    return SSAMD_OK;
}

int ssamd_asw_kernel_form(int width, int rows, int winSize, int maxDisparity, int minDisparity, int *out)
{
    int nD, rc = check_geometry_query(width, winSize, maxDisparity, minDisparity, out, &nD);
    if (rc) return rc;
    const Tuning &t = tune();
    AswGeom g;
    if ((rc = asw_choose_geometry(g, PlanOptions{t, false}, width, rows, winSize, nD))) return rc;
    out[0] = g.pipe; out[1] = g.Rx; out[2] = g.JC >= winSize ? 0 : g.JC; out[3] = g.pipe ? g.dephase : 0;
    out[4] = g.wave_rx & 15;
    if (g.wave_rx) { out[0] = 0; out[1] = g.wave_rx & 15; out[2] = 0; out[3] = 0; }
    return SSAMD_OK;
}

int ssamd_gsw_geometry(int width, int rows, int winSize, int maxDisparity, int minDisparity, int *out)
{
    int nD, rc = check_geometry_query(width, winSize, maxDisparity, minDisparity, out, &nD);
    if (rc) return rc;
    GswGeom g;
    if ((rc = gsw_choose_geometry(g, tune(), width, rows, winSize, nD))) return rc;
    out[0] = g.Tx; out[1] = g.Dc; out[2] = g.nchunks; out[3] = g.threads * g.Hy; out[4] = g.lds_bytes;
    out[5] = (width + g.Tx - 1) / g.Tx; out[6] = (rows + g.Ty * g.Hy - 1) / (g.Ty * g.Hy); out[7] = g.nchunks; out[8] = g.Ty * g.Hy;
    return SSAMD_OK;
}

int ssamd_profile_enable(int on)
{
    for (auto &c : g_ctx) {
        std::lock_guard<std::mutex> lk(c.mu);
        c.prof.on = on != 0;
    }
    return SSAMD_OK;
}

int ssamd_profile_reset(void)
{
    DeviceGuard guard;
    for (auto &c : g_ctx) {
        std::lock_guard<std::mutex> lk(c.mu);
        if (c.dev < 0) continue;
        (void)hipSetDevice(c.dev);
        c.prof.drain();
        std::fill(c.prof.ms, c.prof.ms + SSAMD_K_COUNT, 0.0);
        std::fill(c.prof.n, c.prof.n + SSAMD_K_COUNT, 0LL);
    }
    return SSAMD_OK;
}

int ssamd_profile_read(double *ms, long long *launches)
{
    DeviceGuard guard;
    for (int k = 0; k < SSAMD_K_COUNT; ++k) { if (ms) ms[k] = 0; if (launches) launches[k] = 0; }
    for (auto &c : g_ctx) {
        std::lock_guard<std::mutex> lk(c.mu);
        if (c.dev < 0) continue;
        (void)hipSetDevice(c.dev);
        c.prof.drain();
        for (int k = 0; k < SSAMD_K_COUNT; ++k) { if (ms) ms[k] += c.prof.ms[k]; if (launches) launches[k] += c.prof.n[k]; }
    }
    return SSAMD_OK;
}
}
```

### simplestereo_amd/csrc/ssamd_options.h

```cpp
#pragma once

#define SSAMD_OPTIONS(X) \
    X("SSAMD_ASW_GEOM", asw_geom, std::string, "", v, !x.empty())    \
    X("SSAMD_GSW_GEOM", gsw_geom, std::string, "", v, false) \
    X("SSAMD_GSW_PLAIN", gsw_plain, int, 0, atoi(v) != 0 ? 1 : 0, false)    \
    X("SSAMD_ASW_PIPE", asw_pipe, int, -1, atoi(v), x >= 0)    \
    X("SSAMD_ASW_DEPHASE", asw_dephase, int, -1, atoi(v), x >= 0)    \
    X("SSAMD_ASW_EVOL", asw_evol, int, 1, atoi(v), x != 1)    \
    X("SSAMD_ASW_WAVE", asw_wave, int, -1, atoi(v) != 0 ? 1 : 0, x >= 0)    \
    X("SSAMD_ASW_WAVE_RX", wave_rx, int, 0, atoi(v), x != 0)    \
    X("SSAMD_ASW_WAVE_WG", wave_wg, int, 0, std::max(1, std::min(4, atoi(v))), x != 0)    \
    X("SSAMD_ASW_WAVE_UNROLL", wave_unroll, int, 1, atoi(v), false)    \
    X("SSAMD_ASW_WAVE_MERGE", wave_merge, int, 1, atoi(v), x != 1)    \
    X("SSAMD_ASW_STATIC", asw_static, int, 1, atoi(v), x != 1)    \
    X("SSAMD_ASW_EVOL_MAX_MB", evol_max_mb, int, 0, std::max(0, atoi(v)), x != 0)    \
    X("SSAMD_ASW_WAVE_RD", wave_rd, int, 0, atoi(v), x != 0)    \
    X("SSAMD_ASW_NO_E2", no_e2, bool, false, true, x) \
    X("SSAMD_ASW_XOR_ONLY", xor_only, bool, false, true, x) \
    X("SSAMD_MULTI_ALLOW_REPEAT", multi_allow_repeat, bool, false, true, false) \
    X("SSAMD_ALT_QUEUE_CAP", alt_queue_cap, int, 0, std::max(1, atoi(v)), false)    \
    X("SSAMD_AUTOTUNE", autotune_env, int, -2, atoi(v) > 0 ? 1 : (atoi(v) < 0 ? -1 : 0), false)    \
    X("SSAMD_ASW_EVOL_FAIL", evol_fail, int, 0, atoi(v), false)    \
    X("SSAMD_ASW_TAIL", asw_tail, int, -1, atoi(v), false)    \
    X("SSAMD_ASW_PERSIST", asw_persist, int, -1, atoi(v), x > 0)    \
    X("SSAMD_ASW_WAVE_CREG", wave_creg, int, 1, atoi(v), x != 1)    \
    X("SSAMD_ASW_LDS_RELAX", lds_relax, int, 1, atoi(v), x != 1)    \
    X("SSAMD_ASW_PREPASS_FUSE", prepass_fuse, int, 1, atoi(v), false)    \
    X("SSAMD_EXACT_TOL", exact_tol, int, 128, std::max(0, atoi(v)), false)    \
    X("SSAMD_EXACT_CAP", exact_cap, int, 0, std::max(1, atoi(v)), false)    \
    X("SSAMD_EXACT_RAWCAP", exact_rawcap, int, 0, std::max(1, atoi(v)), false)    \
    X("SSAMD_UNWRAP_ROWS", unwrap_rows, int, 0, std::max(0, std::min(UNWRAP_MAX_ROWS, atoi(v))), false)

struct Tuning {
#define X(NAME, MEMBER, TYPE, UNSET, PARSE, FORCES) TYPE MEMBER = UNSET;
    SSAMD_OPTIONS(X)
#undef X
};

bool tuning_assign(Tuning &t, const std::string &name, const char *v)
{
#define X(NAME, MEMBER, TYPE, UNSET, PARSE, FORCES) \
    if (name == NAME) { if (v) t.MEMBER = PARSE; else t.MEMBER = UNSET; return true; }
    SSAMD_OPTIONS(X)
#undef X
    return false;
}

const char *const kTuningNames[] = {
#define X(NAME, MEMBER, TYPE, UNSET, PARSE, FORCES) NAME,
    SSAMD_OPTIONS(X)
#undef X
};

bool asw_geometry_forced(const Tuning &t)
{
#define X(NAME, MEMBER, TYPE, UNSET, PARSE, FORCES) { const TYPE &x = t.MEMBER; (void)x; if (FORCES) return true; }
    SSAMD_OPTIONS(X)
#undef X
    return false;
}
```

Baseline: 11070.

## Batch exact-eval candidates per wave, add reference weight tables, tile TAD prepass

The exact ASW evaluation now processes four queued candidates per wave, each with its own LDS row pair, and reduces them in parallel lanes rather than with two lanes. A new refmark kernel marks the right reference pixels used by queue entries so their support-weight tables are precomputed and reused instead of recomputing exp/sqrt per tap. The weight-table kernel splits each window across four waves, and the prepass gains a 16-column tiled TAD path. The changes add extra kernels, atomics and LDS use, and alter flag semantics (the R flag is now tested with a bit mask), which carries some correctness risk.

Result: no change. 11100 (median of 6 runs) (+0.3%).

```diff
diff --git a/simplestereo_amd/csrc/asw_exact_kernels.hip.h b/simplestereo_amd/csrc/asw_exact_kernels.hip.h
--- a/simplestereo_amd/csrc/asw_exact_kernels.hip.h
+++ b/simplestereo_amd/csrc/asw_exact_kernels.hip.h
@@ -20,6 +20,7 @@
     uint32_t *wpix;
     double *wtab;
     unsigned int wcap;
+    unsigned char *refR;
     int H, W, win, pad, minD, maxD, row0, rows;
     double gammaC;
 };
@@ -245,9 +246,9 @@
     }
 }
 
-__device__ __forceinline__ void exact_assign_wslot(const AswExactArgs &A, bool flagged, u64 mask, uint32_t pix, uint32_t side)
-{
-    if (mask == 0 || A.wcap == 0) return;
+__device__ __forceinline__ unsigned exact_assign_wslot(const AswExactArgs &A, bool flagged, u64 mask, uint32_t pix, uint32_t side)
+{
+    if (mask == 0 || A.wcap == 0) return 0xffffffffu;
     const int leader = (int)__builtin_ctzll(mask);
     const unsigned lane = __builtin_amdgcn_mbcnt_hi(~0u, __builtin_amdgcn_mbcnt_lo(~0u, 0u));
     unsigned base = 0;
@@ -257,7 +258,9 @@
         const unsigned slot = base + (unsigned)__builtin_popcountll(mask & (((u64)1 << lane) - 1));
         (side ? A.wslotR : A.wslotL)[pix] = slot;
         if (slot < A.wcap) A.wpix[slot] = pix | (side << 31);
-    }
+        return slot;
+    }
+    return 0xffffffffu;
 }
 
 __global__ __launch_bounds__(256) void asw_exact_winners_kernel(const AswExactArgs A)
@@ -294,6 +297,30 @@
     }
 }
 
+__global__ __launch_bounds__(256) void asw_exact_refmark_kernel(const AswExactArgs A, const int left)
+{
+    if (exact_overflowed(A)) return;
+    const unsigned n = min(A.q.counter[0], A.q.cap);
+    const unsigned nloop = (n + 255u) & ~255u;
+    for (unsigned e0 = blockIdx.x * blockDim.x; e0 < nloop; e0 += gridDim.x * blockDim.x) {
+        const unsigned e = e0 + threadIdx.x;
+        bool need = false;
+        uint32_t rp = 0;
+        if (e < n) {
+            const u64 ent = A.q.entries[e];
+            rp = left ? (uint32_t)ent : (uint32_t)ent - (uint32_t)((ent >> 32) & 0xffff);
+            const uintptr_t a = reinterpret_cast<uintptr_t>((left ? A.q.flagL : A.refR) + rp);
+            const unsigned sh = 8u * (unsigned)(a & 3);
+            const unsigned old = atomicOr(reinterpret_cast<unsigned int *>(a & ~(uintptr_t)3), (left ? 1u : 2u) << sh) >> sh;
+            need = (old & 3u) == 0u;
+        }
+        const unsigned slot = exact_assign_wslot(A, need, __builtin_amdgcn_ballot_w64(need), rp, left ? 0u : 1u);
+        const u64 got = __builtin_amdgcn_ballot_w64(need && slot < A.wcap);
+        if (got && (int)__builtin_ctzll(got) == (int)(threadIdx.x & 63)) atomicAdd(A.q.counter + (left ? 1 : 3), (unsigned)__builtin_popcountll(got));
+    }
+}
+
+static constexpr int EXACT_WTAB_PARTS = 4, EXACT_WTAB_BLOCKS = 256 * 8;
 __global__ __launch_bounds__(256) void asw_exact_wtab_kernel(const AswExactArgs A)
 {
 #pragma clang fp contract(off)
@@ -303,14 +330,15 @@
     if (exact_overflowed(A)) return;
     const unsigned n = min(A.q.counter[6], A.wcap);
     const int lane = threadIdx.x & 63, W = A.W, H = A.H, win = A.win, p = A.pad, win2 = win * win;
-    for (unsigned slot = blockIdx.x * 4 + (threadIdx.x >> 6); slot < n; slot += gridDim.x * 4) {
+    for (unsigned it = blockIdx.x * 4 + (threadIdx.x >> 6); it < n * EXACT_WTAB_PARTS; it += gridDim.x * 4) {
+        const unsigned slot = it / EXACT_WTAB_PARTS, part = it % EXACT_WTAB_PARTS;
         const uint32_t pw = A.wpix[slot], pix = pw & 0x7fffffffu;
         const double *const lab = (pw >> 31) ? A.labR : A.labL;
         const int yr = (int)(pix / (uint32_t)W), x = (int)(pix - (uint32_t)yr * (uint32_t)W), y = A.row0 + yr;
         const double *const c = lab + 3 * ((size_t)y * W + x);
         const double c0 = c[0], c1 = c[1], c2 = c[2];
         double *const out = A.wtab + (size_t)slot * win2;
-        for (int t = lane; t < win2; t += 64) {
+        for (int t = (int)part * 64 + lane; t < win2; t += 64 * EXACT_WTAB_PARTS) {
             const int i = t / win, j = t - i * win, ii = y - p + i, cc = x - p + j;
             double w = 0.0;
             if ((unsigned)ii < (unsigned)H && (unsigned)cc < (unsigned)W) {
@@ -324,74 +352,118 @@
 }
 
 static constexpr int EXACT_WAVES = 4;
-static constexpr int EXACT_CHUNK = 256;
+static constexpr int EXACT_G = 4;
+static constexpr int EXACT_CHUNK = 128;
+static constexpr int EXACT_ROW = EXACT_CHUNK + 4;
+static constexpr int EXACT_GROUPS_PER_CU = 3;
+
+struct ExactCand {
+    uint32_t pix;
+    int d, y, x, xr, jlo, ncol, ilo, ntap;
+    float rncol;
+    unsigned flags;
+};
+__device__ __forceinline__ ExactCand exact_decode(const AswExactArgs &A, u64 ent)
+{
+    ExactCand c;
+    c.pix = (uint32_t)ent;
+    c.d = (int)((ent >> 32) & 0xffff);
+    c.flags = (unsigned)(ent >> 48);
+    const int W = A.W, H = A.H, win = A.win, p = A.pad;
+    const int yr = (int)(c.pix / (uint32_t)W);
+    c.x = (int)(c.pix - (uint32_t)yr * (uint32_t)W);
+    c.y = A.row0 + yr;
+    c.xr = c.x - c.d;
+    c.jlo = max(0, p - c.xr);
+    c.ncol = min(win, W + p - c.x) - c.jlo;
+    c.ilo = max(0, p - c.y);
+    c.ntap = (min(win, H + p - c.y) - c.ilo) * c.ncol;
+    c.rncol = 1.0f / (float)max(c.ncol, 1);
+    return c;
+}
+__device__ __forceinline__ int exact_tap_row(const ExactCand &c, int t) { return (int)(((float)t + 0.5f) * c.rncol); }
+
 __global__ __launch_bounds__(64 * EXACT_WAVES) void asw_exact_eval_kernel(const AswExactArgs A)
 {
 #pragma clang fp contract(off)
-    __shared__ double s_w[EXACT_WAVES][EXACT_CHUNK], s_c[EXACT_WAVES][EXACT_CHUNK];
+    __shared__ double s_rows[EXACT_WAVES][2 * EXACT_G][EXACT_ROW];
     __shared__ uint64_t s_exp[256];
     for (int k = threadIdx.x; k < 256; k += blockDim.x) s_exp[k] = gm_exp_tab[k];
     __syncthreads();
     if (exact_overflowed(A)) return;
     const int lane = threadIdx.x & 63, wv = threadIdx.x >> 6;
-    double *const sw = s_w[wv], *const sc = s_c[wv];
     const unsigned n = min(A.q.counter[0], A.q.cap);
-    const int W = A.W, H = A.H, win = A.win, p = A.pad;
-    for (unsigned e = blockIdx.x * EXACT_WAVES + wv; e < n; e += gridDim.x * EXACT_WAVES) {
-        const u64 ent = A.q.entries[e];
-        const uint32_t pix = (uint32_t)ent;
-        const int d = (int)((ent >> 32) & 0xffff);
-        const unsigned sides = (unsigned)(ent >> 48) & 3u;
-        const int yr = (int)(pix / (uint32_t)W), x = (int)(pix - (uint32_t)yr * (uint32_t)W);
-        const int y = A.row0 + yr, xr = x - d;
-        const double *const cl = A.labL + 3 * ((size_t)y * W + x), *const cr = A.labR + 3 * ((size_t)y * W + xr);
-        const double cl0 = cl[0], cl1 = cl[1], cl2 = cl[2], cr0 = cr[0], cr1 = cr[1], cr2 = cr[2];
-        const int jlo = max(0, p - xr), jhi = min(win, W + p - x), ncol = jhi - jlo;
-        const int ilo = max(0, p - y), ihi = min(win, H + p - y);
-        const int ntap = (ihi - ilo) * ncol;
-        const uint32_t s1 = A.wcap && A.q.flagL && A.q.flagL[pix] ? A.wslotL[pix] : 0xffffffffu;
-        const uint32_t s2 = A.wcap && A.q.flagR && A.q.flagR[pix - (uint32_t)d] ? A.wslotR[pix - (uint32_t)d] : 0xffffffffu;
-        const double *const t1 = s1 < A.wcap ? A.wtab + (size_t)s1 * win * win : nullptr;
-        const double *const t2 = s2 < A.wcap ? A.wtab + (size_t)s2 * win * win : nullptr;
+    const int W = A.W, win = A.win, p = A.pad;
+    for (unsigned e0 = (blockIdx.x * EXACT_WAVES + wv) * EXACT_G; e0 < n; e0 += gridDim.x * EXACT_WAVES * EXACT_G) {
+        const int ng = (int)min((unsigned)EXACT_G, n - e0);
+        ExactCand C[EXACT_G];
+        const double *t1[EXACT_G], *t2[EXACT_G];
+        int ntap[EXACT_G];
+        int maxtap = 0;
+#pragma unroll
+        for (int g = 0; g < EXACT_G; ++g) {
+            ntap[g] = 0;
+            t1[g] = t2[g] = nullptr;
+            C[g] = ExactCand{};
+            if (g >= ng) continue;
+            const ExactCand c = exact_decode(A, A.q.entries[e0 + g]);
+            C[g] = c;
+            const uint32_t rpix = c.pix - (uint32_t)c.d;
+            const uint32_t s1 = A.wcap && A.q.flagL && A.q.flagL[c.pix] ? A.wslotL[c.pix] : 0xffffffffu;
+            const uint32_t s2 = A.wcap && A.refR && A.refR[rpix] ? A.wslotR[rpix] : 0xffffffffu;
+            t1[g] = s1 < A.wcap ? A.wtab + (size_t)s1 * win * win : nullptr;
+            t2[g] = s2 < A.wcap ? A.wtab + (size_t)s2 * win * win : nullptr;
+            bool all_zero = false;
+            if (c.flags & EXACT_HINT_ZERO) {
+                bool nz = false;
+                for (int t = lane; t < c.ntap; t += 64) {
+                    const int q = exact_tap_row(c, t), i = c.ilo + q, j = c.jlo + (t - q * c.ncol);
+                    const int ii = c.y - p + i, jj = c.xr - p + j, kk = c.x - p + j;
+                    nz = nz || __builtin_amdgcn_sad_u8(A.recL[(size_t)ii * W + kk].bgrx, A.recR[(size_t)ii * W + jj].bgrx, 0u) != 0u;
+                }
+                all_zero = __builtin_amdgcn_ballot_w64(nz) == 0;
+            }
+            ntap[g] = all_zero ? 0 : c.ntap;
+            maxtap = max(maxtap, ntap[g]);
+        }
+        int my_ntap = 0;
+#pragma unroll
+        for (int g = 0; g < EXACT_G; ++g) my_ntap = (lane >> 1) == g ? ntap[g] : my_ntap;
+        const double *const src = s_rows[wv][lane & (2 * EXACT_G - 1)];
         double acc = 0.0;
-        bool all_zero = false;
-        if ((unsigned)(ent >> 48) & EXACT_HINT_ZERO) {
-            bool nz = false;
-            for (int t = lane; t < ntap; t += 64) {
-                const int q = t / ncol, i = ilo + q, j = jlo + (t - q * ncol);
-                const int ii = y - p + i, jj = xr - p + j, kk = x - p + j;
-                nz = nz || __builtin_amdgcn_sad_u8(A.recL[(size_t)ii * W + kk].bgrx, A.recR[(size_t)ii * W + jj].bgrx, 0u) != 0u;
-            }
-            all_zero = __builtin_amdgcn_ballot_w64(nz) == 0;
-        }
-        for (int t0 = 0; t0 < (all_zero ? 0 : ntap); t0 += EXACT_CHUNK) {
-            const int nt = min(EXACT_CHUNK, ntap - t0);
-            for (int t = lane; t < nt; t += 64) {
-                const int q = (t0 + t) / ncol, i = ilo + q, j = jlo + (t0 + t - q * ncol);
-                const int ii = y - p + i, jj = xr - p + j, kk = x - p + j;
-                const double pr = A.prox[i * win + j];
-                double w1, w2;
-                if (t1) w1 = t1[i * win + j];
-                else {
-                    const double *const tl = A.labL + 3 * ((size_t)ii * W + kk);
-                    const double a0 = tl[0] - cl0, a1 = tl[1] - cl1, a2 = tl[2] - cl2;
-                    w1 = pr * glibc_exp_t(-exact_sqrt(a0 * a0 + a1 * a1 + a2 * a2) / A.gammaC, s_exp);
-                }
-                if (t2) w2 = t2[i * win + j];
-                else {
-                    const double *const tr = A.labR + 3 * ((size_t)ii * W + jj);
-                    const double b0 = tr[0] - cr0, b1 = tr[1] - cr1, b2 = tr[2] - cr2;
-                    w2 = pr * glibc_exp_t(-exact_sqrt(b0 * b0 + b1 * b1 + b2 * b2) / A.gammaC, s_exp);
-                }
-                const int tad = min(40, (int)__builtin_amdgcn_sad_u8(A.recL[(size_t)ii * W + kk].bgrx, A.recR[(size_t)ii * W + jj].bgrx, 0u));
-                const double ww = w1 * w2;
-                sw[t] = ww;
-                sc[t] = ww * tad;
+        for (int t0 = 0; t0 < maxtap; t0 += EXACT_CHUNK) {
+#pragma unroll
+            for (int g = 0; g < EXACT_G; ++g) {
+                const ExactCand &c = C[g];
+                const int nt = min(EXACT_CHUNK, ntap[g] - t0);
+                double *const sc = s_rows[wv][2 * g], *const sw = s_rows[wv][2 * g + 1];
+                const double *const cl = A.labL + 3 * ((size_t)c.y * W + c.x), *const cr = A.labR + 3 * ((size_t)c.y * W + c.xr);
+                for (int t = lane; t < nt; t += 64) {
+                    const int q = exact_tap_row(c, t0 + t), i = c.ilo + q, j = c.jlo + (t0 + t - q * c.ncol);
+                    const int ii = c.y - p + i, jj = c.xr - p + j, kk = c.x - p + j;
+                    double w1, w2;
+                    if (t1[g]) w1 = t1[g][i * win + j];
+                    else {
+                        const double *const tl = A.labL + 3 * ((size_t)ii * W + kk);
+                        const double a0 = tl[0] - cl[0], a1 = tl[1] - cl[1], a2 = tl[2] - cl[2];
+                        w1 = A.prox[i * win + j] * glibc_exp_t(-exact_sqrt(a0 * a0 + a1 * a1 + a2 * a2) / A.gammaC, s_exp);
+                    }
+                    if (t2[g]) w2 = t2[g][i * win + j];
+                    else {
+                        const double *const tr = A.labR + 3 * ((size_t)ii * W + jj);
+                        const double b0 = tr[0] - cr[0], b1 = tr[1] - cr[1], b2 = tr[2] - cr[2];
+                        w2 = A.prox[i * win + j] * glibc_exp_t(-exact_sqrt(b0 * b0 + b1 * b1 + b2 * b2) / A.gammaC, s_exp);
+                    }
+                    const int tad = min(40, (int)__builtin_amdgcn_sad_u8(A.recL[(size_t)ii * W + kk].bgrx, A.recR[(size_t)ii * W + jj].bgrx, 0u));
+                    const double ww = w1 * w2;
+                    sw[t] = ww;
+                    sc[t] = ww * tad;
+                }
             }
             __builtin_amdgcn_wave_barrier();
             asm volatile("s_waitcnt lgkmcnt(0)" ::: "memory");
-            if (lane < 2) {
-                const double *const src = lane ? sw : sc;
+            {
+                const int nt = min(EXACT_CHUNK, my_ntap - t0);
                 int t = 0;
                 for (; t + 16 <= nt; t += 16) {
                     double v[16];
@@ -405,13 +477,19 @@
             asm volatile("s_waitcnt lgkmcnt(0)" ::: "memory");
             __builtin_amdgcn_wave_barrier();
         }
-        const double tot = __shfl(acc, 1);
-        if (lane == 0) {
-            const double c = all_zero ? 0.0 : acc / tot;
-            A.ecost[e] = c;
+        const double tot = __shfl(acc, lane | 1);
+        unsigned long long my_ent = 0;
+#pragma unroll
+        for (int g = 0; g < EXACT_G; ++g) my_ent = (lane >> 1) == g ? ((u64)C[g].flags << 48 | (u64)(uint32_t)C[g].d << 32 | C[g].pix) : my_ent;
+        if (lane < 2 * ng && !(lane & 1)) {
+            const uint32_t pix = (uint32_t)my_ent;
+            const uint32_t d = (uint32_t)(my_ent >> 32) & 0xffffu;
+            const unsigned sides = (unsigned)(my_ent >> 48) & 3u;
+            const double c = my_ntap == 0 ? 0.0 : acc / tot;
+            A.ecost[e0 + (unsigned)(lane >> 1)] = c;
             const u64 bits = (u64)__double_as_longlong(c);
             if (sides & EXACT_SIDE_L) atomicMin(A.costL + pix, bits);
-            if (sides & EXACT_SIDE_R) atomicMin(A.costR + (pix - (uint32_t)d), bits);
+            if (sides & EXACT_SIDE_R) atomicMin(A.costR + (pix - d), bits);
         }
     }
 }
@@ -440,8 +518,8 @@
             if (A.keyL) A.keyL[q] = (A.keyL[q] & 0xffffffff00000000ull) | (u64)A.idxL[q];
             else A.disp[q] = (int16_t)A.idxL[q];
         }
-        if (A.keyR && A.q.flagR[q] && A.idxR[q] != 0xffffffffu) A.keyR[q] = (A.keyR[q] & 0xffffffff00000000ull) | (u64)A.idxR[q];
-    }
-}
-
-}
+        if (A.keyR && (A.q.flagR[q] & 1) && A.idxR[q] != 0xffffffffu) A.keyR[q] = (A.keyR[q] & 0xffffffff00000000ull) | (u64)A.idxR[q];
+    }
+}
+
+}
diff --git a/simplestereo_amd/csrc/asw_prepass_kernels.hip.h b/simplestereo_amd/csrc/asw_prepass_kernels.hip.h
--- a/simplestereo_amd/csrc/asw_prepass_kernels.hip.h
+++ b/simplestereo_amd/csrc/asw_prepass_kernels.hip.h
@@ -5,6 +5,94 @@
 namespace ssamd {
 
 static constexpr int TADV_COLS = 64;
+
+struct TadTile16 {
+    int NJ, NP, CL;
+    __host__ __device__ explicit TadTile16(int Se) : NJ(TADV_COLS + Se), NP(NJ + 4), CL(NP + ((NP >> 4) + 1) * 4) {}
+    __host__ __device__ static int padded(int a) { return a + ((a >> 4) << 2); }
+    __host__ __device__ int lds_dwords() const { return TADV_COLS + 4 * CL; }
+};
+static constexpr int TADV16_MIN_SE = 128;
+__host__ __device__ inline bool tadv_tile16(int Se, int rd) { return ((Se >> 2) & 3) == 0 && rd == 4 && Se >= TADV16_MIN_SE; }
+inline size_t tadv_lds_bytes(int Dc, int Se, int rd)
+{
+    const size_t plain = (size_t)(2 * TADV_COLS + Dc) * 4;
+    return tadv_tile16(Se, rd) ? std::max(plain, (size_t)TadTile16(Se).lds_dwords() * 4) : plain;
+}
+
+template <class Pixel>
+__device__ __forceinline__ void asw_tad_tile16(uint32_t *__restrict__ sL, const Pixel &pixel, const void *__restrict__ srcL, const void *__restrict__ srcR,
+                                               unsigned char *__restrict__ evol, int W, int minD, int Dc, int Se, int erows, int evolW,
+                                               int by, int z, int uc0, int u0)
+{
+    const TadTile16 T(Se);
+    uint32_t *const cps = sL + TADV_COLS;
+    const int dlo = minD + z * Dc, P4 = Se >> 4;
+    bool outside = false;
+    for (int k0 = threadIdx.x; k0 < TADV_COLS + T.NJ; k0 += 2 * blockDim.x) {
+        uint32_t v[2];
+#pragma unroll
+        for (int u = 0; u < 2; ++u) {
+            const int k = k0 + u * (int)blockDim.x;
+            const bool isL = k < TADV_COLS;
+            const int col = isL ? u0 + k : u0 + 2 * TADV_COLS - 1 - dlo - k;
+            v[u] = k < TADV_COLS + T.NJ && (unsigned)col < (unsigned)W ? pixel(isL ? srcL : srcR, col) : 0x80000000u;
+        }
+#pragma unroll
+        for (int u = 0; u < 2; ++u) {
+            const int k = k0 + u * (int)blockDim.x;
+            if (k >= TADV_COLS + T.NJ) continue;
+            outside = outside || (v[u] >> 31);
+            if (k < TADV_COLS) sL[k] = v[u];
+            else {
+#pragma unroll
+                for (int m = 0; m < 4; ++m) cps[m * T.CL + TadTile16::padded(k - TADV_COLS + m)] = v[u];
+            }
+        }
+    }
+    const bool border = __syncthreads_or(outside) != 0;
+    const int ncols = min(TADV_COLS, evolW - uc0);
+    uint4 *const out4 = reinterpret_cast<uint4 *>(evol + (((size_t)z * erows + by) * (size_t)evolW + uc0) * Se);
+    auto item = [&](int c, int blk, auto mode) {
+        constexpr int MODE = decltype(mode)::value;
+        const uint32_t lp = sL[c];
+        const int m = (c + 1) & 3, a0 = (TADV_COLS - 1) - c + 16 * blk + m;
+        const uint32_t *const cp = cps + m * T.CL;
+        uint32_t o[4];
+#pragma unroll
+        for (int i = 0; i < 4; ++i) {
+            const uint4 rv4 = *reinterpret_cast<const uint4 *>(cp + TadTile16::padded(a0 + 4 * i));
+            const uint32_t rv[4] = {rv4.x, rv4.y, rv4.z, rv4.w};
+            const int left = Dc - 16 * blk - 4 * i;
+            uint32_t v = 0;
+#pragma unroll
+            for (int q = 0; q < 4; ++q) {
+                const uint32_t e = min(__builtin_amdgcn_sad_u8(lp, rv[q], 0u), 40u) << (8 * q);
+                if (MODE != 2) v |= e;
+                else if (!(rv[q] >> 31) && q < left) v |= e;
+            }
+            if (MODE == 1) v = left >= 4 ? v : (left > 0 ? v & ((1u << (8 * left)) - 1u) : 0u);
+            if (MODE == 2 && (lp >> 31)) v = 0;
+            o[i] = v;
+        }
+        out4[c * P4 + blk] = make_uint4(o[0], o[1], o[2], o[3]);
+    };
+    auto run = [&](int b0, int nb, auto mode) {
+        const float rnb = 1.0f / (float)max(nb, 1);
+        for (int k = threadIdx.x; k < ncols * nb; k += blockDim.x) {
+            const int c = (int)(((float)k + 0.5f) * rnb);
+            item(c, b0 + k - c * nb, mode);
+        }
+    };
+    if (border) {
+        run(0, P4, std::integral_constant<int, 2>{});
+    } else {
+        const int full = min(P4, Dc >> 4);
+        run(0, full, std::integral_constant<int, 0>{});
+        run(full, P4 - full, std::integral_constant<int, 1>{});
+    }
+}
+
 template <bool BYTES>
 __device__ __forceinline__ void asw_tad_tile(const void *__restrict__ srcL, const void *__restrict__ srcR, unsigned char *__restrict__ evol,
                                              int W, int pad, int minD, int Dc, int Se, int erow0, int erows, int evolW, int rd, long long npix_total,
@@ -26,6 +114,10 @@
             return reinterpret_cast<const PixRec *>(src)[q].bgrx;
         }
     };
+    if (tadv_tile16(Se, rd)) {
+        asw_tad_tile16(sL, pixel, srcL, srcR, evol, W, minD, Dc, Se, erows, evolW, by, z, uc0, u0);
+        return;
+    }
     for (int k = threadIdx.x; k < 2 * TADV_COLS + Dc; k += blockDim.x) {
         const bool isL = k < TADV_COLS;
         const int col = isL ? u0 + k : xr0 + (k - TADV_COLS);
diff --git a/simplestereo_amd/csrc/host_asw.h b/simplestereo_amd/csrc/host_asw.h
--- a/simplestereo_amd/csrc/host_asw.h
+++ b/simplestereo_amd/csrc/host_asw.h
@@ -252,7 +252,7 @@
     const int rd = g.wave_rx ? r.wave.RD : 4;
     Timed t(c, s, SSAMD_K_LAB);
     const dim3 egrid((unsigned)((evolW + TADV_COLS - 1) / TADV_COLS), (unsigned)erows, (unsigned)chunks);
-    const size_t elds = (size_t)(2 * TADV_COLS + Dc) * 4;
+    const size_t elds = tadv_lds_bytes(Dc, Se, rd);
     const long long tiles = (long long)egrid.x * egrid.y * egrid.z;
     if (r.lab_pending && tiles + r.lab_blocks < (1ll << 31)) {
         AswPrepassArgs pa;
diff --git a/simplestereo_amd/csrc/host_asw_exact.h b/simplestereo_amd/csrc/host_asw_exact.h
--- a/simplestereo_amd/csrc/host_asw_exact.h
+++ b/simplestereo_amd/csrc/host_asw_exact.h
@@ -47,6 +47,14 @@
     return SSAMD_OK;
 }
 
+size_t exact_wtab_cap(int win, size_t nout)
+{
+    size_t wcap = std::min<size_t>(65536, ((size_t)64 << 20) / ((size_t)win * win * 8));
+    if (nout >= ((size_t)1 << 31) || tune().exact_wtab == 0) wcap = 0;
+    if (tune().exact_wcap) wcap = std::min<size_t>(wcap, (size_t)tune().exact_wcap);
+    return wcap;
+}
+
 int asw_exact_pass(Ctx &c, const AswExactQueue &q, const AswExactQueue &raw, int H, int W, int row0, int rows, int win, int maxD, int minD, double gammaC, double gammaP,
                    bool consistent, bool direct, int16_t *d_disp, hipStream_t s)
 {
@@ -70,8 +78,7 @@
     x.wslotL = x.idxR + nout; x.wslotR = x.wslotL + nout;
     {
         const size_t per = (size_t)win * win * 8;
-        size_t wcap = std::min<size_t>(65536, ((size_t)64 << 20) / per);
-        if (nout >= ((size_t)1 << 31)) wcap = 0;
+        size_t wcap = exact_wtab_cap(win, nout);
         if (wcap && (rc = c.xwtab.reserve(wcap * 8 + wcap * per))) return rc;
         x.wcap = (unsigned int)wcap;
         x.wpix = (uint32_t *)c.xwtab.ptr;
@@ -79,6 +86,7 @@
     }
     x.H = H; x.W = W; x.win = win; x.pad = p; x.minD = minD; x.maxD = maxD; x.row0 = row0; x.rows = rows;
     x.gammaC = gammaC;
+    x.refR = x.wcap ? q.flagL + nout : nullptr;
     Timed t(c, s, SSAMD_K_ASW_EXACT);
     {
         const int r0 = std::max(0, row0 - p), r1 = std::min(H, row0 + rows + p);
@@ -100,8 +108,9 @@
         hipLaunchKernelGGL(asw_exact_zero_kernel, dim3((unsigned)std::min<long long>(segs, 256 * 64)), dim3(256), zlds, s, x);
     }
     hipLaunchKernelGGL(asw_exact_winners_kernel, dim3(pb), dim3(256), 0, s, x);
-    if (x.wcap) hipLaunchKernelGGL(asw_exact_wtab_kernel, dim3(256 * 4), dim3(256), 0, s, x);
-    hipLaunchKernelGGL(asw_exact_eval_kernel, dim3((unsigned)(c.cus * 5)), dim3(64 * EXACT_WAVES), 0, s, x);
+    if (x.wcap && tune().exact_wtab >= 2) hipLaunchKernelGGL(asw_exact_refmark_kernel, dim3(256 * 4), dim3(256), 0, s, x, 0);
+    if (x.wcap) hipLaunchKernelGGL(asw_exact_wtab_kernel, dim3(EXACT_WTAB_BLOCKS), dim3(256), 0, s, x);
+    hipLaunchKernelGGL(asw_exact_eval_kernel, dim3((unsigned)(c.cus * EXACT_GROUPS_PER_CU)), dim3(64 * EXACT_WAVES), 0, s, x);
     hipLaunchKernelGGL(asw_exact_resolve_kernel, dim3(256 * 4), dim3(256), 0, s, x);
     hipLaunchKernelGGL(asw_exact_patch_kernel, dim3(pb), dim3(256), 0, s, x);
     HIP_TRY(hipGetLastError());
@@ -112,7 +121,7 @@
 int asw_exact_counters(Ctx &c, unsigned int (&ctr)[5])
 {
     std::fill(ctr, ctr + 5, 0u);
-    if (!c.xflags.ptr || c.exact_calls == 0) return SSAMD_OK;
+    if (!c.xflags.ptr || !c.xcap) return SSAMD_OK;
     HIP_TRY(hipDeviceSynchronize());
     HIP_TRY(hipMemcpy(ctr, c.xflags.ptr, sizeof(ctr), hipMemcpyDeviceToHost));
     return SSAMD_OK;
diff --git a/simplestereo_amd/csrc/host_context.h b/simplestereo_amd/csrc/host_context.h
--- a/simplestereo_amd/csrc/host_context.h
+++ b/simplestereo_amd/csrc/host_context.h
@@ -135,7 +135,7 @@
     bool lut_ready = false;
     hipStream_t stream = nullptr;
     DevBuf imgL, imgR, recL, recR, keyL, keyR, disp, costs, lab, altq, evol, altdisp;
-    DevBuf xlabL, xlabR, xflags, xqueue, xcost, xslots, xctr, xraw, xwtab;
+    DevBuf xlabL, xlabR, xflags, xqueue, xcost, xslots, xraw, xwtab;
     DevBuf pq;
     DevBuf uwIn, uwOut;
     DevBuf ftpBand, ftpPhase;
diff --git a/simplestereo_amd/csrc/host_debug.h b/simplestereo_amd/csrc/host_debug.h
--- a/simplestereo_amd/csrc/host_debug.h
+++ b/simplestereo_amd/csrc/host_debug.h
@@ -36,8 +36,10 @@
     ScratchOrder order(*c, s);
     if ((rc = c->imgL.reserve(npix * 3)) || (rc = c->imgR.reserve(npix * 3)) || (rc = c->recL.reserve(npix * sizeof(PixRec))) ||
         (rc = c->recR.reserve(npix * sizeof(PixRec))) || (rc = c->xlabL.reserve(npix * 24)) || (rc = c->xlabR.reserve(npix * 24)) ||
-        (rc = c->xqueue.reserve((size_t)std::max(n, 1) * 8)) || (rc = c->xcost.reserve((size_t)std::max(n, 1) * 8)) || (rc = c->xctr.reserve(64)))
+        (rc = c->xqueue.reserve((size_t)std::max(n, 1) * 8)) || (rc = c->xcost.reserve((size_t)std::max(n, 1) * 8)) ||
+        (rc = c->xflags.reserve(64 + 2 * npix + 4)) || (rc = c->xslots.reserve(npix * 8)))
         return rc;
+    if (npix >= ((size_t)1 << 31)) return fail(SSAMD_ELIMIT, "more than 2^31 pixels");
     HIP_TRY(hipMemcpyAsync(c->imgL.ptr, img1, npix * 3, hipMemcpyHostToDevice, s));
     HIP_TRY(hipMemcpyAsync(c->imgR.ptr, img2, npix * 3, hipMemcpyHostToDevice, s));
     const int blocks = (int)std::min<long long>((2 * (long long)npix + 255) / 256, 256 * 8);
@@ -53,15 +55,31 @@
     }
     const unsigned int ctr[16] = {(unsigned int)n};
     HIP_TRY(hipMemcpyAsync(c->xqueue.ptr, ent.data(), (size_t)n * 8, hipMemcpyHostToDevice, s));
-    HIP_TRY(hipMemcpyAsync(c->xctr.ptr, ctr, sizeof(ctr), hipMemcpyHostToDevice, s));
+    HIP_TRY(hipMemsetAsync(c->xflags.ptr, 0, 64 + 2 * npix + 4, s));
+    HIP_TRY(hipMemcpyAsync(c->xflags.ptr, ctr, sizeof(ctr), hipMemcpyHostToDevice, s));
+    c->xcap = (unsigned int)std::max(n, 1);
+    c->xrawcap = 0;
     const double *d_prox = nullptr;
     if ((rc = get_prox64(*c, winSize, gammaP, s, &d_prox))) return rc;
     AswExactArgs x{};
     x.recL = (const PixRec *)c->recL.ptr; x.recR = (const PixRec *)c->recR.ptr;
     x.labL = (const double *)c->xlabL.ptr; x.labR = (const double *)c->xlabR.ptr;
-    x.prox = d_prox; x.q.entries = (u64 *)c->xqueue.ptr; x.q.counter = (unsigned int *)c->xctr.ptr; x.q.cap = (unsigned int)std::max(n, 1);
+    x.prox = d_prox; x.q.entries = (u64 *)c->xqueue.ptr; x.q.counter = (unsigned int *)c->xflags.ptr; x.q.cap = (unsigned int)std::max(n, 1);
     x.ecost = (double *)c->xcost.ptr;
     x.H = height; x.W = width; x.win = winSize; x.pad = winSize / 2; x.row0 = 0; x.rows = height; x.gammaC = gammaC;
+    const size_t wcap = exact_wtab_cap(winSize, npix), per = (size_t)winSize * winSize * 8;
+    if (wcap) {
+        if ((rc = c->xwtab.reserve(wcap * 8 + wcap * per))) return rc;
+        x.wcap = (unsigned int)wcap;
+        x.wpix = (uint32_t *)c->xwtab.ptr;
+        x.wtab = (double *)((char *)c->xwtab.ptr + wcap * 8);
+        x.wslotL = (uint32_t *)c->xslots.ptr; x.wslotR = x.wslotL + npix;
+        x.q.flagL = (unsigned char *)c->xflags.ptr + 64;
+        x.refR = x.q.flagL + npix;
+        hipLaunchKernelGGL(asw_exact_refmark_kernel, dim3(256), dim3(256), 0, s, x, 1);
+        if (tune().exact_wtab >= 2) hipLaunchKernelGGL(asw_exact_refmark_kernel, dim3(256), dim3(256), 0, s, x, 0);
+        hipLaunchKernelGGL(asw_exact_wtab_kernel, dim3(EXACT_WTAB_BLOCKS), dim3(256), 0, s, x);
+    }
     hipLaunchKernelGGL(asw_exact_eval_kernel, dim3(256), dim3(64 * EXACT_WAVES), 0, s, x);
     HIP_TRY(hipGetLastError());
     HIP_TRY(hipMemcpyAsync(costs, c->xcost.ptr, (size_t)n * 8, hipMemcpyDeviceToHost, s));
diff --git a/simplestereo_amd/csrc/host_library.h b/simplestereo_amd/csrc/host_library.h
--- a/simplestereo_amd/csrc/host_library.h
+++ b/simplestereo_amd/csrc/host_library.h
@@ -68,11 +68,11 @@
         }
         *value = (long long)done;
     }
-    else if (n == "exact_entries" || n == "exact_flagged_left" || n == "exact_flagged_right" || n == "exact_overflow" || n == "exact_raw_entries") {
+    else if (n == "exact_entries" || n == "exact_flagged_left" || n == "exact_flagged_right" || n == "exact_overflow" || n == "exact_raw_entries" || n == "exact_wtab_right") {
         unsigned int ctr[5];
         if ((rc = asw_exact_counters(*c, ctr))) return rc;
         *value = n == "exact_entries" ? ctr[0] : n == "exact_flagged_left" ? ctr[1] : n == "exact_flagged_right" ? ctr[2] :
-                 n == "exact_raw_entries" ? ctr[4] : ((ctr[0] > c->xcap || (c->xrawcap && ctr[4] > c->xrawcap)) ? 1 : 0);
+                 n == "exact_raw_entries" ? ctr[4] : n == "exact_wtab_right" ? ctr[3] : ((ctr[0] > c->xcap || (c->xrawcap && ctr[4] > c->xrawcap)) ? 1 : 0);
     }
     else return fail(SSAMD_EINVAL, "unknown counter %s", name);
     return SSAMD_OK;
diff --git a/simplestereo_amd/csrc/ssamd_options.h b/simplestereo_amd/csrc/ssamd_options.h
--- a/simplestereo_amd/csrc/ssamd_options.h
+++ b/simplestereo_amd/csrc/ssamd_options.h
@@ -29,6 +29,8 @@
     X("SSAMD_EXACT_TOL", exact_tol, int, 128, std::max(0, atoi(v)), false)    \
     X("SSAMD_EXACT_CAP", exact_cap, int, 0, std::max(1, atoi(v)), false)    \
     X("SSAMD_EXACT_RAWCAP", exact_rawcap, int, 0, std::max(1, atoi(v)), false)    \
+    X("SSAMD_EXACT_WTAB", exact_wtab, int, 2, std::max(0, std::min(2, atoi(v))), false)    \
+    X("SSAMD_EXACT_WCAP", exact_wcap, int, 0, std::max(1, atoi(v)), false)    \
     X("SSAMD_UNWRAP_ROWS", unwrap_rows, int, 0, std::max(0, std::min(UNWRAP_MAX_ROWS, atoi(v))), false)
 
 struct Tuning {
```
